# baldhat/yolov10-3D

Measured on AMD Instinct MI355X. Metric: train_images_per_sec, higher is better.
Workload: dtype bf16

## Files before the change

include/y3d.h:

```cpp
#ifndef Y3D_H
#define Y3D_H
#include <stdint.h>

#ifdef __cplusplus
extern "C" {
#endif

enum { Y3D_F32 = 0, Y3D_BF16 = 1 };
enum { Y3D_OK = 0, Y3D_ERR_INVALID = -1, Y3D_ERR_HIP = -2 };

const char* y3d_last_error(void);
int y3d_abi_version(void);
int y3d_device_info(char* name, int name_len, int* compute_units, int* lds_bytes, int* clock_khz);

int y3d_pack_weight_fwd(int dtype, const float* w_oihw, void* out, int Cout, int Cin_g, int Cin_g_pad, int kh, int kw, void* stream);
int y3d_pack_weight_dgrad(int dtype, const float* w_oihw, void* out, int Cout, int Cin_g, int groups, int kh, int kw, void* stream);
int y3d_mt_pack_weights(int dtype, const int64_t* desc, const int* chunk_tensor, const int* chunk_off, int nchunks, int chunk, void* stream);
int y3d_mt_fp8w_quantize(const int64_t* desc, const int* row_begin, int ntensors, int nrows, void* stream);
int y3d_fp8w_dequantize(const uint8_t* codes, const float* scale, float* w, int rows, int K, void* stream);
int y3d_fp8_quantize_act(const void* x, int64_t xsw, int64_t M, int C, uint8_t* q, uint8_t* s, void* stream);
int y3d_fp8_pack_weight_fwd(const uint8_t* codes, const float* scale, int rows, int Cg, uint8_t* wq, uint8_t* ws, void* stream);
int y3d_conv3x3_fp8_ok(int B, int H, int W, int Cin, int Cout, int groups);
int y3d_conv3x3_fp8_stat_rows(int B, int H, int W);
int y3d_fp8_scale_pitch(int C);
int y3d_conv3x3_fp8_fwd(const uint8_t* xq, const uint8_t* xs, int B, int H, int W, int Cin, const uint8_t* wq, const uint8_t* ws, void* y, int64_t ysw,
                        int Cout, int groups, float* stat_partials, const float* scale, const float* shift, int act, void* stream);
int y3d_fp8_quantize_grad(const void* dy, int64_t sw, const float* scale, int64_t M, int C, uint8_t* q, uint8_t* s, void* stream);
int y3d_fp8_pack_weight_dgrad(const uint8_t* codes, int Cout, int Cin, int groups, int lo, int hi, uint8_t* wq, uint8_t* ws, void* stream);
int y3d_conv3x3_fp8_dgrad_ok(int B, int H, int W, int Cin, int Cout, int groups);
int y3d_conv3x3_fp8_dgrad(const uint8_t* dyq, const uint8_t* dys, int64_t qsw, int spitch, int lo, int hi, int B, int H, int W, const uint8_t* wq, const uint8_t* ws,
                          void* dx, int64_t dxsw, int Cin, int groups, void* stream);
int y3d_conv_kpad(int dtype, int k_total);
int y3d_conv_stat_blocks(int B, int Ho, int Wo);
int y3d_conv2d_stat_rows(int dtype, int B, int H, int W, int Cin, int Cout, int groups, int kh, int kw, int stride, int pad);
enum { Y3D_OP_FWD = 0, Y3D_OP_BWD_DATA = 1, Y3D_OP_BWD_WEIGHT = 2 };
enum { Y3D_EPI_RAW = 0, Y3D_EPI_PARTIALS = 1, Y3D_EPI_AFFINE = 2, Y3D_EPI_AFFINE_RES = 3, Y3D_EPI_BIAS = 4 };
enum {
  Y3D_ROUTE_GENERIC = 0,
  Y3D_ROUTE_STREAM1X1 = 1,
  Y3D_ROUTE_SMALL = 2,
  Y3D_ROUTE_SMALL_S2 = 3,
  Y3D_ROUTE_S2_DGRAD = 4,
  Y3D_ROUTE_TILE8 = 5,
  Y3D_ROUTE_TILE16 = 6,
  Y3D_ROUTE_WIDE3_8 = 7,
  Y3D_ROUTE_WIDE3_16 = 8,
  Y3D_ROUTE_FLAT = 9,
  Y3D_ROUTE_WGRAD_SMALL = 10,
  Y3D_ROUTE_WGRAD_TILE = 11,
  Y3D_ROUTE_WGRAD_STREAM1X1 = 12
};
int y3d_conv2d_route(int dtype, int op, int epi, int B, int H, int W, int Cin, int Cout, int groups, int kh, int kw, int stride, int pad);
int y3d_conv2d_fwd(int dtype, const void* x, int64_t xsb, int64_t xsh, int64_t xsw, int B, int H, int W, int Cin,
                   const void* w_packed, const float* bias, void* y, int64_t ysw, int Ho, int Wo, int Cout, int groups,
                   int kh, int kw, int stride, int pad, float* stat_partials, void* stream);
int y3d_conv2d_fwd_affine(int dtype, const void* x, int64_t xsb, int64_t xsh, int64_t xsw, int B, int H, int W, int Cin,
                          const void* w_packed, const float* scale, const float* shift, int act, void* y, int64_t ysw, int Ho, int Wo,
                          int Cout, int groups, int kh, int kw, int stride, int pad, void* stream);
int y3d_conv2d_fwd_affine_res_ok(int dtype, int B, int H, int W, int Cin, int Cout, int groups, int kh, int kw, int stride, int pad);
int y3d_conv2d_fwd_affine_res(int dtype, const void* x, int64_t xsb, int64_t xsh, int64_t xsw, int B, int H, int W, int Cin,
                              const void* w_packed, const float* scale, const float* shift, int act, const void* res, int64_t rsw, void* y,
                              int64_t ysw, int Ho, int Wo, int Cout, int groups, int kh, int kw, int stride, int pad, void* stream);
int y3d_conv2d_bwd_data(int dtype, const void* dy, int64_t dsb, int64_t dsh, int64_t dsw, int B, int Ho, int Wo, int Cout,
                        const void* w_packed_dgrad, void* dx, int64_t xsw, int H, int W, int Cin, int groups, int kh, int kw,
                        int stride, int pad, void* stream);
int y3d_conv2d_wgrad_splits(int dtype, int B, int Ho, int Wo, int Cout, int Cin_g, int groups, int kh, int kw);
int y3d_conv2d_wgrad_plan(int dtype, int B, int H, int W, int Cin, int Cout, int groups, int kh, int kw, int stride, int pad);
int y3d_set_tile_kernels(int enable);
int y3d_set_stream1x1(int enable);
int y3d_get_stream1x1(void);
int y3d_get_tile_kernels(void);
int y3d_set_bn_wide_slabs(int enable);
int y3d_conv2d_bwd_weight(int dtype, const void* x, int64_t xsb, int64_t xsh, int64_t xsw, int B, int H, int W, int Cin,
                          int Cin_real, const void* dy, int64_t dsw, int Ho, int Wo, int Cout, int groups, int kh, int kw,
                          int stride, int pad, float* slab, int nsplit, float* grad_oihw, int accumulate, void* stream);

int y3d_dw_blocks(int64_t M);
int y3d_dw_wgrad_blocks(int64_t M);
int y3d_dw_pack_weight(const float* w_oihw, float* out_taps_c, int C, int kh, int kw, void* stream);
int y3d_dwconv2d_fwd(int dtype, const void* x, int64_t xsb, int64_t xsh, int64_t xsw, int B, int H, int W, int C,
                     const float* w_packed, void* y, int64_t ysw, int Ho, int Wo, int kh, int kw, int stride, int pad,
                     float* stat_partials, void* stream);
int y3d_dwconv2d_fwd_affine(int dtype, const void* x, int64_t xsb, int64_t xsh, int64_t xsw, int B, int H, int W, int C,
                            const float* w_packed, const float* scale, const float* shift, int act, int res_mode, const void* res, int64_t rsw,
                            void* z, int64_t zsw, int Ho, int Wo, int kh, int kw, int stride, int pad, void* stream);
int y3d_dwconv2d_bwd_data(int dtype, const void* dy, int64_t dsb, int64_t dsh, int64_t dsw, int B, int Ho, int Wo, int C,
                          const float* w_packed, void* dx, int64_t xsw, int H, int W, int kh, int kw, int stride, int pad,
                          void* stream);
int y3d_dwconv2d_bwd_weight(int dtype, const void* x, int64_t xsb, int64_t xsh, int64_t xsw, int B, int H, int W, int C,
                            const void* dy, int64_t dsw, int Ho, int Wo, int kh, int kw, int stride, int pad, float* slab,
                            float* grad_oihw, int accumulate, void* stream);

int y3d_bn_finalize(const float* partials, int nblk, int C, int64_t count, const float* gamma, const float* beta, float eps,
                    float momentum, float* running_mean, float* running_var, float* mean, float* invstd, float* scale,
                    float* shift, void* stream);
int y3d_bn_eval_scale(int C, const float* gamma, const float* beta, const float* running_mean, const float* running_var,
                      float eps, float* scale, float* shift, void* stream);
int y3d_bn_act_fwd(int dtype, const void* y, int64_t ysw, const float* scale, const float* shift, int act, int res_mode,
                   const void* res, int64_t rsw, void* z, int64_t zsw, int64_t P, int C, void* stream);
int y3d_bn_act_fwd_q(const void* y, int64_t ysw, const float* scale, const float* shift, int act, void* z, int64_t zsw, uint8_t* q, uint8_t* s,
                     int64_t P, int C, void* stream);
int y3d_bn_bwd_blocks(int64_t P, int C);
int y3d_bn_act_bwd_reduce(int dtype, const void* y, int64_t ysw, const void* dz, int64_t dsw, const void* res, int64_t rsw,
                          const float* scale, const float* shift, const float* mean, const float* invstd, int act,
                          int res_mode, float* partials, int64_t P, int C, void* stream);
int y3d_bn_bwd_finalize(const float* partials, int nblk, int C, int64_t count, float* dgamma, float* dbeta, int accumulate,
                        float* mean_g, float* mean_gx, void* stream);
int y3d_bn_act_bwd_apply(int dtype, const void* y, int64_t ysw, const void* dz, int64_t dsw, const void* res, int64_t rsw,
                         const float* scale, const float* shift, const float* mean, const float* invstd,
                         const float* mean_g, const float* mean_gx, int act, int res_mode, int train, void* dy, int64_t dysw,
                         void* dres, int64_t drsw, int64_t P, int C, void* stream);
int y3d_colsum_partials(int dtype, const void* x, int64_t xsw, float* partials, int64_t P, int C, void* stream);

int y3d_maxpool_fwd(int dtype, const void* x, int64_t xsb, int64_t xsh, int64_t xsw, void* y, int64_t ysw, uint8_t* argmax,
                    int B, int H, int W, int C, int k, void* stream);
int y3d_maxpool_bwd(int dtype, const void* dy, int64_t dsw, const uint8_t* argmax, void* dx, int64_t xsw, int B, int H, int W,
                    int C, int k, void* stream);
int y3d_upsample2x_fwd(int dtype, const void* x, int64_t xsb, int64_t xsh, int64_t xsw, void* y, int64_t ysw, int B, int H, int W,
                       int C, void* stream);
int y3d_upsample2x_bwd(int dtype, const void* dy, int64_t dsb, int64_t dsh, int64_t dsw, void* dx, int64_t xsw, int B, int H,
                       int W, int C, void* stream);
int y3d_copy2d(int dtype, const void* x, int64_t xsw, void* y, int64_t ysw, int64_t P, int C, void* stream);
int y3d_occupy_cus(int n, const int* flag, float* buf, int64_t nbuf, void* stream);
int y3d_add2d(int dtype, const void* a, int64_t asw, const void* b, int64_t bsw, void* y, int64_t ysw, int64_t P, int C, void* stream);
int y3d_nchw_to_nhwc(int dtype, const float* x_nchw, void* y_nhwc, int B, int C, int H, int W, int Cpad, void* stream);
int y3d_stem_im2col(int dtype, const float* x_nchw, void* out, int B, int H, int W, int Ho, int Wo, void* stream);
int y3d_stem_im2col_u8(int dtype, const uint8_t* x, int hwc, void* out, int B, int H, int W, int Ho, int Wo, void* stream);
int y3d_stem_conv_eval(const void* x, int in_mode, const float* wcol, const float* scale, const float* shift, int act, void* y, int64_t ysw,
                       int B, int H, int W, int Cout, void* stream);
int y3d_stem_conv_train_rows(int B, int H, int W);
int y3d_stem_conv_train(const void* x, int in_mode, const float* wcol, void* y, int64_t ysw, void* xcol, float* part, int B, int H, int W,
                        int Cout, void* stream);
int y3d_nhwc_to_nchw(int dtype, const void* x_nhwc, int64_t xsw, float* y_nchw, int B, int C, int H, int W, void* stream);
int y3d_proj_fwd(int dtype, const void* x, int64_t xsw, const float* w, const float* bias, void* y, int64_t ysw, int64_t P,
                 int Cin, int Cout, void* stream);
int y3d_proj_bwd_data(int dtype, const void* dy, int64_t dsw, const float* w, void* dx, int64_t xsw, int64_t P, int Cin, int Cout,
                      void* stream);
int y3d_proj_blocks(int64_t P);
int y3d_proj_bwd_weight(int dtype, const void* x, int64_t xsw, const void* dy, int64_t dsw, float* slab, float* bias_slab,
                        float* grad_w, float* grad_b, int accumulate, int64_t P, int Cin, int Cout, void* stream);
int y3d_slab_reduce(const float* slab, float* out, int nblk, int64_t n, int accumulate, void* stream);
int y3d_proj_group_fwd(int dtype, int nb, int cin, const void* x, int64_t xsw, const int* xoff, const float* const* w,
                       const float* const* b, const int* couts, void* y, int64_t ysw, int64_t P, void* stream);
int y3d_proj_group_bwd_data(int dtype, int nb, int cin, const void* dy, int64_t dsw, const int* xoff, const float* const* w,
                            const int* couts, void* dx, int64_t xsw, int64_t P, void* stream);
int y3d_proj_group_fwd_bn_mfma(int nb, int cin, const void* y_pre, int64_t ysw, const int* xoff, const float* const* w, const float* const* b,
                               const int* couts, const float* scale, const float* shift, int act, void* out, int64_t osw, int64_t P,
                               void* stream);
int y3d_proj_group_bwd_weight_bn_mfma_blocks(int64_t P);
int y3d_proj_group_bwd_weight_bn_mfma(int nb, int cin, const void* y_pre, int64_t ysw, const int* xoff, const void* dout, int64_t dsw,
                                      const int* couts, const float* scale, const float* shift, int act, float* slab, float* bslab,
                                      float* const* dw, float* const* db, int64_t P, void* stream);
int y3d_proj_group_bn_bwd_blocks(int64_t P);
int y3d_proj_group_bn_bwd(int mode, int nb, int cin, const void* y_pre, int64_t ysw, const int* xoff, const void* dout, int64_t dsw,
                          const float* const* w, const int* couts, const float* scale, const float* shift, const float* mean,
                          const float* invstd, const float* mean_g, const float* mean_gx, int act, float* partials, int nblk, void* dy,
                          int64_t dysw, int64_t P, int C, void* stream);
int y3d_proj_group_blocks(int64_t P);
int y3d_proj_group_fwd_bn(int dtype, int nb, int cin, const void* y_pre, int64_t xsw, const int* xoff, const float* const* w,
                          const float* const* b, const int* couts, const float* scale, const float* shift, int act, void* out,
                          int64_t ysw, int64_t P, void* stream);
int y3d_proj_group_bwd_weight_bn(int dtype, int nb, int cin, const void* y_pre, int64_t xsw, const int* xoff, const void* dy, int64_t dsw,
                                 const int* couts, const float* scale, const float* shift, int act, float* slab, float* bslab,
                                 float* const* dw, float* const* db, int64_t P, void* stream);
int y3d_proj_group_bwd_weight(int dtype, int nb, int cin, const void* x, int64_t xsw, const int* xoff, const void* dy, int64_t dsw,
                              const int* couts, float* slab, float* bslab, float* const* dw, float* const* db, int64_t P, void* stream);

int y3d_attn_fwd(int dtype, const void* qkv, int64_t qsw, void* out, int64_t osw, float* lse, int B, int N, int nh, int kd, int hd,
                 float scale, void* stream);
int y3d_attn_bwd(int dtype, const void* qkv, int64_t qsw, const void* out, int64_t osw, const void* dout, int64_t dsw,
                 const void* dv_extra, int64_t esw, const float* lse, float* delta, void* dqkv, int64_t gsw, int B, int N, int nh,
                 int kd, int hd, float scale, void* stream);

int y3d_tal3d_scratch_floats(int B, int n, int A, int topk);
int y3d_pad_targets(const float* rows, int nbox, int width, int B, int cap, float scale_x, float scale_y, float* out, int* n_used,
                    void* stream);
int y3d_tal3d_assign(int dtype, int nl, const void* const* maps, const int64_t* psw, const int* H, const int* W, const float* strides,
                     int B, int nc, const float* gt, int n, const float* calib, const float* mean_sizes, int topk, float alpha,
                     float beta, float gamma, int mode, float* scratch, uint8_t* fg_mask, int* target_gt_idx, float* target_scores, float* scal,
                     const int* n_used, void* stream);
int y3d_loss3d(int dtype, int nl, const void* const* maps, const int64_t* psw, void* const* grads, const int64_t* gsw, const int* H,
               const int* W, const float* strides, int B, int nc, const float* gt, int n, const uint8_t* fg_mask,
               const int* target_gt_idx, const float* target_scores, const float* scal, float w_loss2d, float w_cls, float w_depth,
               float w_offset3d, float w_size3d, float w_heading, float grad_scale, float* partials, float* items, void* stream);

int y3d_distill_loss(int dtype, int nl, const void* const* embs, const int64_t* psw, const int* H, const int* W, int B, int C,
                     const void* teacher, int teacher_dtype, int th, int tw, int64_t tsb, int64_t tsc, int64_t tsh, int64_t tsw,
                     const float* gt, int n, const uint8_t* fg_mask, const int* target_gt_idx, const float* scal, const uint8_t* mixed,
                     int img_w, int img_h, float T, float weight, int criterion, int no_mixup, int cap, int* counts, int* idx,
                     void* rows, float* partials, float* loss, void* stream);
int y3d_distill_scatter(int dtype, const void* rows, const int* idx, const int* nrows, const float* scale, int cap, int C, void* grad,
                        int64_t sb, int64_t sh, int64_t sw, int a0, int H, int W, void* stream);

int y3d_tal2d_assign(int dtype, int nl, const void* const* maps, const int64_t* psw, const int* H, const int* W, const float* strides,
                     int B, int nc, const float* gt, int n, int topk, float alpha, float beta, float* scratch, uint8_t* fg_mask,
                     int* target_gt_idx, float* target_scores, float* scal, const int* n_used, void* stream);
int y3d_loss2d(int dtype, int nl, const void* const* maps, const int64_t* psw, void* const* grads, const int64_t* gsw, const int* H,
               const int* W, const float* strides, int B, int nc, const float* gt, int n, const uint8_t* fg_mask,
               const int* target_gt_idx, const float* target_scores, const float* scal, float w_box, float w_cls, float w_dfl,
               float grad_scale, float* partials, float* items, void* stream);
int y3d_tal2d_scratch_floats(int B, int n, int A, int topk);
int y3d_tal2d_assign_crowded(int dtype, int nl, const void* const* maps, const int64_t* psw, const int* H, const int* W, const float* strides,
                             int B, int nc, const float* gt, int n, int topk, float alpha, float beta, float* scratch, uint8_t* fg_mask,
                             int* target_gt_idx, float* target_scores, float* scal, const int* n_used, void* stream);

int y3d_topk_cells(int dtype, const void* cls, int64_t psw, int B, int HW, int nc, int K, int* out_idx, void* stream);
int y3d_patch_gather(int dtype, const void* x, int64_t xsb, int64_t xsh, int64_t xsw, const int* idx, void* out, int B, int H, int W,
                     int C, int K, int ps, void* stream);
int y3d_head3d_scatter(int dtype, const void* cls, int64_t csw, const void* reg, int64_t rsw, const int* idx, void* map, int B, int HW,
                       int nc, int no, int K, void* stream);
int y3d_head3d_decode(int dtype, int nl, const void* const* maps, const int* H, const int* W, const float* strides, int B, int nc,
                      float* y, void* stream);
int y3d_head2d_decode(int dtype, int nl, const void* const* maps, const int* H, const int* W, const float* strides, int B, int nc,
                      float* y, void* stream);
int y3d_v10_postprocess_scratch_floats(int B, int A, int nc, int max_det);
int y3d_v10_postprocess(const float* y, int B, int C, int A, int nc, int max_det, int boxes_first, float* reg, float* scores,
                        int64_t* labels, float* scratch, void* stream);

int y3d_kitti_image_aug(const unsigned char* const* src, const unsigned char* const* src2, const int* hw, const int* flip, const double* trans_inv,
                        int B, int out_h, int out_w, int mode, void* out, void* stream);
int y3d_kde_depth_fusion(const float* predsO, int B, int K, const float* predsM, int KM, int C, float thres, float iou_thres, int nprop,
                         float* out, void* stream);
int y3d_kitti_decode(const float* preds, int B, int K, const double* calib, const double* ratio, const double* inv_trans,
                     const double* mean_size, int nc, int use_camera_dis, double threshold, double* out, unsigned char* keep, void* stream);
int y3d_kitti_encode_labels(const double* rec, const int* img_i, const double* img_f, int B, int out_w, int out_h, double min_depth,
                            double max_depth, int use_camera_dis, const double* mean_size, int n_cls, int max_objs, int64_t* cls,
                            double* bboxes, float* center_2d, float* size_2d, double* center_3d, double* size_3d, double* depth,
                            int64_t* heading_bin, double* heading_res, float* batch_idx, int* counts, double* calib, double* ratio_pad,
                            void* stream);
int y3d_json3d_encode_labels(const double* rec, const int* img_i, const double* img_f, int B, int dataset, int out_w, int out_h,
                             double min_depth, double max_depth, int use_camera_dis, const double* mean_size, int n_cls, int max_objs,
                             int64_t* cls, double* bboxes, float* center_2d, float* size_2d, double* center_3d, double* size_3d,
                             double* depth, int64_t* heading_bin, double* heading_res, float* batch_idx, int* counts, double* calib,
                             double* ratio_pad, void* stream);
int y3d_yolo2d_image_aug(const unsigned char* const* src, int n_src, const int* rec_i, const double* rec_f, const unsigned char* lut, int B,
                         int imgsz, int mode, void* out, void* stream);
int y3d_yolo2d_encode_labels(const float* rec, int n_rec, const int* lab_i, const float* lab_f, int B, int imgsz, int cap, float* cls,
                             float* bboxes, float* batch_idx, int* counts, void* stream);

int y3d_kitti_eval_max_boxes(void);
int y3d_kitti_box_overlaps(int metric, const float* gt, const float* dt, const int* gt_off, const int* dt_off, const int64_t* ov_off,
                           int n_img, float* out, void* stream);
int y3d_kitti_eval_thresholds(const float* gt, const int* gt_code, const float* dt, const int* dt_code, const int* gt_off, const int* dt_off,
                              const int64_t* ov_off, const float* ov, int n_img, int total_gt, int metric, const int* cd, int ncd,
                              const double* min_ov, int nk, float* tp_score, int* nvalid, void* stream);
int y3d_kitti_eval_counts(const float* gt, const int* gt_code, const float* dt, const int* dt_code, const int* gt_off, const int* dt_off,
                          const int64_t* ov_off, const float* ov, int n_img, int metric, const int* cd, int ncd, const double* min_ov, int nk,
                          const float* thr, const int* nthr, int compute_aos, int* cnt, double* sim, double* pr, void* stream);

int y3d_det_metrics_max_gts(void);
int y3d_det_metrics_max_dets(void);
int y3d_box_iou(const float* box1, int n1, const float* box2, int n2, float eps, float* out, void* stream);
int y3d_match_predictions(const float* iou, const int* gt_cls, int n_gt, const int* det_cls, int n_det, const float* thr, int n_thr,
                          int* tp, void* stream);
int y3d_box_match_batch(int mode, const void* preds, const unsigned char* keep, int B, int K, const double* meta, int img_h, int img_w,
                        int single_cls, const float* gt_img, const float* gt_cls, const float* gt_box, int n_gt, const float* thr,
                        int n_thr, int* tp, double* conf, int* cls, int* status, void* stream);
int y3d_ap_per_class(const int* tp, const double* conf, const int* cls, int64_t n, const int* ucls, const double* nl, int nc, int n_thr,
                     const double* x_ap, int n_ap, const double* x_curve, int n_curve, double* ap, double* p_curve, double* r_curve,
                     void* stream);

int y3d_mt_sqnorm(const int64_t* grad_ptrs, const int64_t* sizes, const int* chunk_tensor, const int* chunk_off, int nchunks, int chunk,
                  float* partials, void* stream);
int y3d_mt_copy(const int64_t* src_ptrs, const int64_t* dst_ptrs, const int64_t* sizes, const int* chunk_tensor, const int* chunk_off,
                int nchunks, int chunk, float scale, void* stream);
int y3d_mt_clip_coef(const float* partials, int nchunks, float max_norm, float* out_norm_clip, void* stream);
int y3d_mt_sgd(const int64_t* param_ptrs, const int64_t* grad_ptrs, const int64_t* buf_ptrs, const int64_t* sizes, const float* lr,
               const float* wd, const int* chunk_tensor, const int* chunk_off, int nchunks, int chunk, float momentum, int nesterov,
               int first_step, const float* norm_clip, void* stream);

int y3d_mt_adamw(const int64_t* param_ptrs, const int64_t* grad_ptrs, const int64_t* m_ptrs, const int64_t* v_ptrs, const int64_t* sizes,
                 const float* lr, const float* wd, const int* chunk_tensor, const int* chunk_off, int nchunks, int chunk, float beta1, float beta2,
                 float eps, float bias_corr1, float bias_corr2_sqrt, const float* norm_clip, void* stream);
int y3d_mt_ema(const int64_t* ema_ptrs, const int64_t* model_ptrs, const int64_t* sizes, const int* reps, const int* chunk_tensor,
               const int* chunk_off, int nchunks, int chunk, float decay, float one_minus_decay, const float* guard, void* stream);

#ifdef __cplusplus
}
#endif
#endif
```

yolov10-3d_amd/_lib.py:

```python
from __future__ import annotations

import ctypes
import os
import re

_HERE = os.path.dirname(os.path.abspath(__file__))
LIB_PATH = os.path.join(_HERE, "liby3d_hip.so")
HEADER = os.path.join(os.path.dirname(_HERE), "include", "y3d.h")

F32, BF16 = 0, 1

_CT = {"int": ctypes.c_int, "int64_t": ctypes.c_int64, "float": ctypes.c_float, "double": ctypes.c_double}


class Y3DError(RuntimeError):
    pass


def parse_header(path: str = HEADER):
    src = open(path).read()
    src = re.sub(r"/\*.*?\*/", " ", src, flags=re.S)
    protos = {}
    for m in re.finditer(r"(const\s+char\s*\*|int)\s+(y3d_\w+)\s*\(([^;{]*?)\)\s*;", src, flags=re.S):
        ret, name, args = m.group(1), m.group(2), m.group(3).strip()
        argtypes = []
        if args and args != "void":
            for a in args.split(","):
                a = a.strip()
                if "*" in a:
                    argtypes.append(ctypes.c_void_p)
                else:
                    toks = a.split()
                    t = toks[1] if toks[0] == "const" else toks[0]
                    argtypes.append(_CT[t])
        protos[name] = (ctypes.c_char_p if "char" in ret else ctypes.c_int, argtypes)
    return protos


_PLAIN_INT = {"abi_version", "conv_kpad", "conv_stat_blocks", "conv2d_stat_rows", "conv2d_route", "conv2d_wgrad_splits", "conv2d_wgrad_plan", "set_tile_kernels", "set_stream1x1", "set_bn_wide_slabs", "get_stream1x1", "get_tile_kernels", "dw_blocks", "dw_wgrad_blocks", "bn_bwd_blocks", "proj_blocks", "proj_group_blocks", "proj_group_bn_bwd_blocks", "proj_group_bwd_weight_bn_mfma_blocks", "tal3d_scratch_floats", "tal2d_scratch_floats", "v10_postprocess_scratch_floats", "conv2d_fwd_affine_res_ok", "stem_conv_train_rows", "conv3x3_fp8_ok", "conv3x3_fp8_dgrad_ok", "conv3x3_fp8_stat_rows", "fp8_scale_pitch", "kitti_eval_max_boxes", "det_metrics_max_gts", "det_metrics_max_dets"}


class _Lib:
    def __init__(self):
        if not os.path.exists(LIB_PATH):
            raise Y3DError(
                f"{LIB_PATH} not found: build it with `python yolov10-3d_amd/csrc/build.py` "
                "(or __graft_entry__.build()). There is no CPU / PyTorch fallback for the HIP path.")
        self._dll = ctypes.CDLL(LIB_PATH)
        self.protos = parse_header()
        for name, (ret, argtypes) in self.protos.items():
            fn = getattr(self._dll, name)
            fn.restype = ret
            fn.argtypes = argtypes

    def last_error(self) -> str:
        return (self._dll.y3d_last_error() or b"").decode()

    def __getattr__(self, name):
        if name.startswith("_"):
            raise AttributeError(name)
        fn = getattr(self._dll, "y3d_" + name)
        ret = self.protos["y3d_" + name][0]
        if ret is not ctypes.c_int or name in _PLAIN_INT:
            setattr(self, name, fn)
            return fn

        def call(*a):
            rc = fn(*a)
            if rc != 0:
                raise Y3DError(f"y3d_{name} failed ({rc}): {self.last_error()}")
            return rc

        setattr(self, name, call)
        return call


_lib = None


def lib() -> _Lib:
    global _lib
    if _lib is None:
        _lib = _Lib()
    return _lib
```

yolov10-3d_amd/csrc/dwconv.hip:

```cpp
#include "common.h"

namespace {

template <int CE>
__device__ __forceinline__ void pk_fma(float* acc, const float* a, const float* b) {
  typedef float f32x2_t __attribute__((ext_vector_type(2)));
#pragma unroll
  for (int j = 0; j < CE; j += 2) {
    const f32x2_t c2 = {acc[j], acc[j + 1]}, a2 = {a[j], a[j + 1]}, b2 = {b[j], b[j + 1]};
    const f32x2_t o2 = __builtin_elementwise_fma(a2, b2, c2);
    acc[j] = o2[0];
    acc[j + 1] = o2[1];
  }
}

struct DwP {
  const void* x;
  const float* w;
  void* y;
  float* part;
  long xsb, xsh, xsw, ysw;
  int B, Hg, Wg, Hq, Wq, C, kh, kw, stride, pad;
  long M;
  int px_per_block;
  const float *scale, *shift;
  const void* res;
  long rsw;
  int act, res_mode;
};

template <typename T, bool DGRAD, int K, bool AFF = false>
__global__ __launch_bounds__(256) void dwconv_kernel(DwP p) {
  constexpr int CE = TT<T>::CE;
  constexpr int CT = 64 / CE;
  constexpr int PT = 256 / CT;
  extern __shared__ __attribute__((aligned(16))) char smem[];
  float* sw = (float*)smem;
  const int taps = p.kh * p.kw;
  float* sred = sw + taps * 64;
  const int ct = threadIdx.x % CT, pt = threadIdx.x / CT;
  const int cs = blockIdx.y * 64;
  const int c = cs + ct * CE;
  for (int i = threadIdx.x; i < taps * 64; i += 256) {
    int t = i / 64, cc = i % 64;
    sw[i] = (cs + cc < p.C) ? p.w[(long)t * p.C + cs + cc] : 0.f;
  }
  __syncthreads();
  const T* __restrict__ X = (const T*)p.x;
  T* __restrict__ Y = (T*)p.y;
  float s1[CE], s2[CE];
#pragma unroll
  for (int j = 0; j < CE; ++j) { s1[j] = 0.f; s2[j] = 0.f; }
  float esc[CE], esf[CE];
  if (AFF && c < p.C) {
#pragma unroll
    for (int j = 0; j < CE; ++j) { esc[j] = p.scale[c + j]; esf[j] = p.shift[c + j]; }
  }
  if (c < p.C) {
    long pbeg = (long)blockIdx.x * p.px_per_block;
    long pend = pbeg + p.px_per_block < p.M ? pbeg + p.px_per_block : p.M;
    const int HWq = p.Hq * p.Wq;
    for (long m = pbeg + pt; m < pend; m += PT) {
      const int mi = (int)m;
      int b = mi / HWq;
      int rem = mi - b * HWq;
      int hq = rem / p.Wq, wq = rem - hq * p.Wq;
      float acc[CE];
#pragma unroll
      for (int j = 0; j < CE; ++j) acc[j] = 0.f;
      const T* xb = X + (long)b * p.xsb + c;
      if (K == 3 && DGRAD && p.stride == 2) {
        const int r0 = (hq + p.pad) & 1, q0 = (wq + p.pad) & 1;
        uint4 raw[2][2];
        int tapi[2][2];
#pragma unroll
        for (int rr = 0; rr < 2; ++rr) {
          const int r = r0 + 2 * rr, th = hq + p.pad - r, hh = th >> 1;
          const bool okh = r < 3 && th >= 0 && hh < p.Hg;
#pragma unroll
          for (int qq = 0; qq < 2; ++qq) {
            const int q = q0 + 2 * qq, tw = wq + p.pad - q, ww = tw >> 1;
            const bool ok = okh && q < 3 && tw >= 0 && ww < p.Wg;
            raw[rr][qq] = ok ? *(const uint4*)(xb + (long)hh * p.xsh + (long)ww * p.xsw) : make_uint4(0, 0, 0, 0);
            tapi[rr][qq] = ok ? r * 3 + q : 0;
          }
        }
#pragma unroll
        for (int rr = 0; rr < 2; ++rr)
#pragma unroll
          for (int qq = 0; qq < 2; ++qq) {
            float v[CE];
            Chunk<T>::unpack(raw[rr][qq], v);
            pk_fma<CE>(acc, v, sw + tapi[rr][qq] * 64 + ct * CE);
          }
      } else if (K > 0) {
#pragma unroll K == 3 ? 3 : 1
        for (int r = 0; r < K; ++r) {
          int hh;
          bool okh;
          if (DGRAD) { int t = hq + p.pad - r; hh = t / p.stride; okh = t >= 0 && hh * p.stride == t && hh < p.Hg; }
          else { hh = hq * p.stride - p.pad + r; okh = hh >= 0 && hh < p.Hg; }
          uint4 raw[K > 0 ? K : 1];
#pragma unroll
          for (int q = 0; q < K; ++q) {
            int ww;
            bool okw;
            if (DGRAD) { int t = wq + p.pad - q; ww = t / p.stride; okw = t >= 0 && ww * p.stride == t && ww < p.Wg; }
            else { ww = wq * p.stride - p.pad + q; okw = ww >= 0 && ww < p.Wg; }
            raw[q] = (okh && okw) ? *(const uint4*)(xb + (long)hh * p.xsh + (long)ww * p.xsw) : make_uint4(0, 0, 0, 0);
          }
#pragma unroll
          for (int q = 0; q < K; ++q) {
            float v[CE];
            Chunk<T>::unpack(raw[q], v);
            pk_fma<CE>(acc, v, sw + (r * K + q) * 64 + ct * CE);
          }
        }
      } else
      for (int r = 0; r < p.kh; ++r) {
        int hh;
        bool okh;
        if (DGRAD) { int t = hq + p.pad - r; hh = t / p.stride; okh = t >= 0 && hh * p.stride == t && hh < p.Hg; }
        else { hh = hq * p.stride - p.pad + r; okh = hh >= 0 && hh < p.Hg; }
        if (!okh) continue;
        for (int q = 0; q < p.kw; ++q) {
          int ww;
          bool okw;
          if (DGRAD) { int t = wq + p.pad - q; ww = t / p.stride; okw = t >= 0 && ww * p.stride == t && ww < p.Wg; }
          else { ww = wq * p.stride - p.pad + q; okw = ww >= 0 && ww < p.Wg; }
          if (!okw) continue;
          float v[CE];
          Chunk<T>::unpack(*(const uint4*)(xb + (long)hh * p.xsh + (long)ww * p.xsw), v);
          pk_fma<CE>(acc, v, sw + (r * p.kw + q) * 64 + ct * CE);
        }
      }
#pragma unroll
      for (int j = 0; j < CE; ++j) {
        acc[j] = TT<T>::rnd(acc[j]);
        s1[j] += acc[j];
        s2[j] += acc[j] * acc[j];
      }
      if (AFF) {
        float r[CE];
        if (p.res_mode) Chunk<T>::unpack(*(const uint4*)((const T*)p.res + m * p.rsw + c), r);
#pragma unroll
        for (int j = 0; j < CE; ++j) {
          float u = acc[j] * esc[j] + esf[j];
          if (p.res_mode == 2) u += r[j];
          if (p.act) u = silu_f(u);
          if (p.res_mode == 1) u += r[j];
          acc[j] = u;
        }
      }
      *(uint4*)(Y + m * p.ysw + c) = Chunk<T>::pack(acc);
    }
  }
  if (p.part) {
#pragma unroll
    for (int j = 0; j < CE; ++j) { sred[(pt * 64 + ct * CE + j) * 2] = s1[j]; sred[(pt * 64 + ct * CE + j) * 2 + 1] = s2[j]; }
    __syncthreads();
    if (threadIdx.x < 64 && cs + threadIdx.x < p.C) {
      float a = 0.f, b2 = 0.f;
      for (int r = 0; r < PT; ++r) { a += sred[(r * 64 + threadIdx.x) * 2]; b2 += sred[(r * 64 + threadIdx.x) * 2 + 1]; }
      p.part[((long)blockIdx.x * p.C + cs + threadIdx.x) * 2] = a;
      p.part[((long)blockIdx.x * p.C + cs + threadIdx.x) * 2 + 1] = b2;
    }
  }
}

struct DwWP {
  const void* x;
  const void* dy;
  float* slab;
  long xsb, xsh, xsw, dsw;
  int B, H, W, Ho, Wo, C, kh, kw, stride, pad;
  long M;
  int px_per_block, nblk, nslab;
};

template <typename T, int K>
__global__ __launch_bounds__(256) void dwconv_wgrad_kernel(DwWP p) {
  constexpr int CE = TT<T>::CE;
  constexpr int CT = 64 / CE;
  constexpr int PT = 256 / CT;
  constexpr int RP = 1;
  constexpr int KW = K > 0 ? K : 8;
  __shared__ float sh[4][RP * KW * 64];
  const int ct = threadIdx.x % CT, pt = threadIdx.x / CT;
  const int kh = K > 0 ? K : p.kh, kw = K > 0 ? K : p.kw;
  const int L = blockIdx.x, jx = L >> 3;
  const int row = jx % kh, tile = (jx / kh) * 8 + (L & 7);
  if (tile >= p.nblk * p.nslab) return;
  const int bx = tile % p.nblk;
  const int cs = (tile / p.nblk) * 64;
  const int c = cs + ct * CE;
  const int taps = kh * kw;
  const T* __restrict__ X = (const T*)p.x;
  const T* __restrict__ D = (const T*)p.dy;
  const long pbeg = (long)bx * p.px_per_block;
  const long pend = pbeg + p.px_per_block < p.M ? pbeg + p.px_per_block : p.M;
  const int HWo = p.Ho * p.Wo;
  {
    const int r0 = row * RP;
    float acc[RP][KW][CE];
#pragma unroll
    for (int r = 0; r < RP; ++r)
#pragma unroll
      for (int q = 0; q < KW; ++q)
#pragma unroll
        for (int j = 0; j < CE; ++j) acc[r][q][j] = 0.f;
    if (c < p.C) {
      long m = pbeg + pt;
      int b = (int)(m / HWo);
      int rem = (int)(m - (long)b * HWo);
      int ho = rem / p.Wo, wo = rem - ho * p.Wo;
      auto one = [&](const uint4& dv, int bb, int hh0, int ww0) {
        float d[CE];
        Chunk<T>::unpack(dv, d);
        const T* xb = X + (long)bb * p.xsb + c;
        uint4 raw[RP][KW];
#pragma unroll
        for (int r = 0; r < RP; ++r) {
          const int hh = hh0 + r0 + r;
          const bool okh = r0 + r < kh && hh >= 0 && hh < p.H;
#pragma unroll
          for (int q = 0; q < KW; ++q) {
            const int ww = ww0 + q;
            const bool ok = okh && q < kw && ww >= 0 && ww < p.W;
            raw[r][q] = ok ? *(const uint4*)(xb + (long)hh * p.xsh + (long)ww * p.xsw) : make_uint4(0, 0, 0, 0);
          }
        }
#pragma unroll
        for (int r = 0; r < RP; ++r)
#pragma unroll
          for (int q = 0; q < KW; ++q) {
            float v[CE];
            Chunk<T>::unpack(raw[r][q], v);
            pk_fma<CE>(acc[r][q], d, v);
          }
      };
      auto advance = [&]() {
        wo += PT;
        while (wo >= p.Wo) { wo -= p.Wo; ++ho; }
        while (ho >= p.Ho) { ho -= p.Ho; ++b; }
      };
      for (; m + PT < pend; m += 2 * PT) {
        const uint4 d0 = *(const uint4*)(D + m * p.dsw + c), d1 = *(const uint4*)(D + (m + PT) * p.dsw + c);
        const int b0 = b, h0 = ho * p.stride - p.pad, w0 = wo * p.stride - p.pad;
        advance();
        const int b1 = b, h1 = ho * p.stride - p.pad, w1 = wo * p.stride - p.pad;
        advance();
        one(d0, b0, h0, w0);
        one(d1, b1, h1, w1);
      }
      if (m < pend) one(*(const uint4*)(D + m * p.dsw + c), b, ho * p.stride - p.pad, wo * p.stride - p.pad);
    }
    const int lane = threadIdx.x & 63, wave = threadIdx.x >> 6;
#pragma unroll
    for (int r = 0; r < RP; ++r)
#pragma unroll
      for (int q = 0; q < KW; ++q)
#pragma unroll
        for (int j = 0; j < CE; ++j) {
          float v = acc[r][q][j];
          if (CT == 8) v = lane_xor8_sum(v);
          v = lane_xor32_sum(lane_xor16_sum(v));
          if (lane < CT) sh[wave][(r * KW + q) * 64 + ct * CE + j] = v;
        }
    __syncthreads();
    for (int i = threadIdx.x; i < RP * KW * 64; i += 256) {
      const int t = i >> 6, cc = i & 63;
      const int r = t / KW, q = t - r * KW;
      if (r0 + r < kh && q < kw && cs + cc < p.C)
        p.slab[((long)bx * taps + (r0 + r) * kw + q) * p.C + cs + cc] = sh[0][i] + sh[1][i] + sh[2][i] + sh[3][i];
    }
  }
}

__global__ __launch_bounds__(256) void dw_wgrad_reduce_kernel(const float* __restrict__ slab, float* __restrict__ grad, int nblk, int taps, int C,
                                                              int accumulate) {
  __shared__ float sh[8][32];
  const int e = threadIdx.x & 31, sl = threadIdx.x >> 5;
  const int idx = blockIdx.x * 32 + e;
  const int n = taps * C;
  float s = 0.f;
  if (idx < n)
    for (int b = sl; b < nblk; b += 8) s += slab[(long)b * n + idx];
  sh[sl][e] = s;
  __syncthreads();
  if (sl != 0 || idx >= n) return;
#pragma unroll
  for (int j = 1; j < 8; ++j) s += sh[j][e];
  const int c = idx % C, t = idx / C;
  const long o = (long)c * taps + t;
  grad[o] = accumulate ? grad[o] + s : s;
}

__global__ void dw_pack_kernel(const float* __restrict__ w, float* __restrict__ out, int C, int taps) {
  int idx = blockIdx.x * blockDim.x + threadIdx.x;
  if (idx >= taps * C) return;
  int c = idx % C, t = idx / C;
  out[idx] = w[(long)c * taps + t];
}

}

extern "C" {

int y3d_dw_blocks(int64_t M) {
  long n = (M + 63) / 64;
  return (int)(n < 1 ? 1 : (n > 2048 ? 2048 : n));
}

int y3d_dw_wgrad_blocks(int64_t M) {
  long n = (M + 127) / 128;
  return (int)(n < 1 ? 1 : (n > 1024 ? 1024 : n));
}

int y3d_dw_pack_weight(const float* w_oihw, float* out, int C, int kh, int kw, void* stream) {
  hipLaunchKernelGGL(dw_pack_kernel, dim3(cdiv((long)C * kh * kw, 256)), dim3(256), 0, (hipStream_t)stream, w_oihw, out, C, kh * kw);
  Y3D_LAUNCH_CHECK();
  return Y3D_OK;
}

#define DW_LAUNCH_K(T, D, K) hipLaunchKernelGGL((dwconv_kernel<T, D, K>), grid, dim3(256), sm, st, p)
#define DW_LAUNCH_A(T, K) hipLaunchKernelGGL((dwconv_kernel<T, false, K, true>), grid, dim3(256), sm, st, p)
#define DW_LAUNCH(T)                                                                                             \
  do {                                                                                                           \
    const int kk = (p.kh == p.kw && (p.kh == 3 || p.kh == 7)) ? p.kh : 0;                                        \
    if (!dgrad && p.scale) { if (kk == 3) DW_LAUNCH_A(T, 3); else if (kk == 7) DW_LAUNCH_A(T, 7); else DW_LAUNCH_A(T, 0); }           \
    else if (dgrad) { if (kk == 3) DW_LAUNCH_K(T, true, 3); else if (kk == 7) DW_LAUNCH_K(T, true, 7); else DW_LAUNCH_K(T, true, 0); }     \
    else { if (kk == 3) DW_LAUNCH_K(T, false, 3); else if (kk == 7) DW_LAUNCH_K(T, false, 7); else DW_LAUNCH_K(T, false, 0); }        \
  } while (0)

static int dw_launch(int dtype, bool dgrad, const DwP& p, hipStream_t st) {
  Y3D_CHECK(p.M < (1L << 31), "dwconv: more than 2^31 pixels");
  int ce = dtype == Y3D_BF16 ? 8 : 4;
  int pt = 256 / (64 / ce);
  size_t sm = (size_t)(p.kh * p.kw * 64 + pt * 64 * 2) * sizeof(float);
  dim3 grid(y3d_dw_blocks(p.M), cdiv(p.C, 64));
  if (dtype == Y3D_BF16) {
    DW_LAUNCH(bf16_t);
  } else {
    DW_LAUNCH(float);
  }
  Y3D_LAUNCH_CHECK();
  return Y3D_OK;
}

int y3d_dwconv2d_fwd(int dtype, const void* x, int64_t xsb, int64_t xsh, int64_t xsw, int B, int H, int W, int C,
                     const float* w_packed, void* y, int64_t ysw, int Ho, int Wo, int kh, int kw, int stride, int pad,
                     float* stat_partials, void* stream) {
  int ce = dtype == Y3D_BF16 ? 8 : 4;
  Y3D_CHECK(dtype == Y3D_BF16 || dtype == Y3D_F32, "dwconv2d_fwd: bad dtype");
  Y3D_CHECK(C % ce == 0, "dwconv2d_fwd: C=%d not a multiple of %d", C, ce);
  Y3D_CHECK(Ho == (H + 2 * pad - kh) / stride + 1 && Wo == (W + 2 * pad - kw) / stride + 1, "dwconv2d_fwd: output dims");
  Y3D_CHECK((((uintptr_t)x | (uintptr_t)y) & 15) == 0 && xsb % ce == 0 && xsh % ce == 0 && xsw % ce == 0 && ysw % ce == 0, "dwconv2d_fwd: alignment");
  DwP p;
  p.x = x; p.w = w_packed; p.y = y; p.part = stat_partials;
  p.scale = nullptr; p.shift = nullptr; p.res = nullptr; p.rsw = 0; p.act = 0; p.res_mode = 0;
  p.xsb = xsb; p.xsh = xsh; p.xsw = xsw; p.ysw = ysw;
  p.B = B; p.Hg = H; p.Wg = W; p.Hq = Ho; p.Wq = Wo; p.C = C; p.kh = kh; p.kw = kw; p.stride = stride; p.pad = pad;
  p.M = (long)B * Ho * Wo;
  int nblk = y3d_dw_blocks(p.M);
  p.px_per_block = (int)((p.M + nblk - 1) / nblk);
  return dw_launch(dtype, false, p, (hipStream_t)stream);
}

int y3d_dwconv2d_fwd_affine(int dtype, const void* x, int64_t xsb, int64_t xsh, int64_t xsw, int B, int H, int W, int C,
                            const float* w_packed, const float* scale, const float* shift, int act, int res_mode, const void* res, int64_t rsw,
                            void* z, int64_t zsw, int Ho, int Wo, int kh, int kw, int stride, int pad, void* stream) {
  int ce = dtype == Y3D_BF16 ? 8 : 4;
  Y3D_CHECK(dtype == Y3D_BF16 || dtype == Y3D_F32, "dwconv2d_fwd_affine: bad dtype");
  Y3D_CHECK(C % ce == 0, "dwconv2d_fwd_affine: C=%d not a multiple of %d", C, ce);
  Y3D_CHECK(Ho == (H + 2 * pad - kh) / stride + 1 && Wo == (W + 2 * pad - kw) / stride + 1, "dwconv2d_fwd_affine: output dims");
  Y3D_CHECK((((uintptr_t)x | (uintptr_t)z) & 15) == 0 && xsb % ce == 0 && xsh % ce == 0 && xsw % ce == 0 && zsw % ce == 0, "dwconv2d_fwd_affine: alignment");
  Y3D_CHECK(scale && shift && res_mode >= 0 && res_mode <= 2, "dwconv2d_fwd_affine: scale / shift missing or bad residual mode");
  Y3D_CHECK(res_mode == 0 || (res && (((uintptr_t)res) & 15) == 0 && rsw % ce == 0), "dwconv2d_fwd_affine: residual missing or misaligned");
  DwP p;
  p.x = x; p.w = w_packed; p.y = z; p.part = nullptr;
  p.scale = scale; p.shift = shift; p.res = res; p.rsw = rsw; p.act = act; p.res_mode = res_mode;
  p.xsb = xsb; p.xsh = xsh; p.xsw = xsw; p.ysw = zsw;
  p.B = B; p.Hg = H; p.Wg = W; p.Hq = Ho; p.Wq = Wo; p.C = C; p.kh = kh; p.kw = kw; p.stride = stride; p.pad = pad;
  p.M = (long)B * Ho * Wo;
  int nblk = y3d_dw_blocks(p.M);
  p.px_per_block = (int)((p.M + nblk - 1) / nblk);
  return dw_launch(dtype, false, p, (hipStream_t)stream);
}

int y3d_dwconv2d_bwd_data(int dtype, const void* dy, int64_t dsb, int64_t dsh, int64_t dsw, int B, int Ho, int Wo, int C,
                          const float* w_packed, void* dx, int64_t xsw, int H, int W, int kh, int kw, int stride, int pad,
                          void* stream) {
  int ce = dtype == Y3D_BF16 ? 8 : 4;
  Y3D_CHECK(dtype == Y3D_BF16 || dtype == Y3D_F32, "dwconv2d_bwd_data: bad dtype");
  Y3D_CHECK(C % ce == 0, "dwconv2d_bwd_data: C=%d not a multiple of %d", C, ce);
  Y3D_CHECK((((uintptr_t)dy | (uintptr_t)dx) & 15) == 0 && dsb % ce == 0 && dsh % ce == 0 && dsw % ce == 0 && xsw % ce == 0, "dwconv2d_bwd_data: alignment");
  DwP p;
  p.x = dy; p.w = w_packed; p.y = dx; p.part = nullptr;
  p.scale = nullptr; p.shift = nullptr; p.res = nullptr; p.rsw = 0; p.act = 0; p.res_mode = 0;
  p.xsb = dsb; p.xsh = dsh; p.xsw = dsw; p.ysw = xsw;
  p.B = B; p.Hg = Ho; p.Wg = Wo; p.Hq = H; p.Wq = W; p.C = C; p.kh = kh; p.kw = kw; p.stride = stride; p.pad = pad;
  p.M = (long)B * H * W;
  int nblk = y3d_dw_blocks(p.M);
  p.px_per_block = (int)((p.M + nblk - 1) / nblk);
  return dw_launch(dtype, true, p, (hipStream_t)stream);
}

int y3d_dwconv2d_bwd_weight(int dtype, const void* x, int64_t xsb, int64_t xsh, int64_t xsw, int B, int H, int W, int C,
                            const void* dy, int64_t dsw, int Ho, int Wo, int kh, int kw, int stride, int pad, float* slab,
                            float* grad_oihw, int accumulate, void* stream) {
  int ce = dtype == Y3D_BF16 ? 8 : 4;
  Y3D_CHECK(dtype == Y3D_BF16 || dtype == Y3D_F32, "dwconv2d_bwd_weight: bad dtype");
  Y3D_CHECK(C % ce == 0, "dwconv2d_bwd_weight: C=%d not a multiple of %d", C, ce);
  Y3D_CHECK((((uintptr_t)x | (uintptr_t)dy) & 15) == 0 && xsb % ce == 0 && xsh % ce == 0 && xsw % ce == 0 && dsw % ce == 0, "dwconv2d_bwd_weight: alignment");
  DwWP p;
  p.x = x; p.dy = dy; p.slab = slab;
  p.xsb = xsb; p.xsh = xsh; p.xsw = xsw; p.dsw = dsw;
  p.B = B; p.H = H; p.W = W; p.Ho = Ho; p.Wo = Wo; p.C = C; p.kh = kh; p.kw = kw; p.stride = stride; p.pad = pad;
  p.M = (long)B * Ho * Wo;
  int nblk = y3d_dw_wgrad_blocks(p.M);
  p.px_per_block = (int)((p.M + nblk - 1) / nblk);
  p.nblk = nblk; p.nslab = cdiv(C, 64);
  dim3 grid(cdiv(nblk * p.nslab, 8) * 8 * kh);
  hipStream_t st = (hipStream_t)stream;
  Y3D_CHECK(kw <= 8 || (kh == kw && (kh == 3 || kh == 7)), "dwconv2d_bwd_weight: kernels wider than 8 taps are not supported");
#define Y3D_DWW(T)                                                                                                          \
  do {                                                                                                                      \
    if (kh == 3 && kw == 3) hipLaunchKernelGGL((dwconv_wgrad_kernel<T, 3>), grid, dim3(256), 0, st, p);                      \
    else if (kh == 7 && kw == 7) hipLaunchKernelGGL((dwconv_wgrad_kernel<T, 7>), grid, dim3(256), 0, st, p);                 \
    else hipLaunchKernelGGL((dwconv_wgrad_kernel<T, 0>), grid, dim3(256), 0, st, p);                                         \
  } while (0)
  if (dtype == Y3D_BF16) Y3D_DWW(bf16_t); else Y3D_DWW(float);
#undef Y3D_DWW
  Y3D_LAUNCH_CHECK();
  hipLaunchKernelGGL(dw_wgrad_reduce_kernel, dim3(cdiv((long)C * kh * kw, 32)), dim3(256), 0, st, slab, grad_oihw, nblk, kh * kw, C, accumulate);
  Y3D_LAUNCH_CHECK();
  return Y3D_OK;
}

}
```

yolov10-3d_amd/ops.py:

```python
from __future__ import annotations

import os
from collections import namedtuple

import torch

from ._lib import BF16, F32, Y3DError, lib

_COMPUTE_DTYPE = torch.bfloat16


def set_compute_dtype(dt: torch.dtype):
    global _COMPUTE_DTYPE
    if dt not in (torch.bfloat16, torch.float32):
        raise ValueError("compute dtype must be torch.bfloat16 or torch.float32")
    _COMPUTE_DTYPE = dt


def compute_dtype() -> torch.dtype:
    return _COMPUTE_DTYPE


def code(dt: torch.dtype) -> int:
    if dt == torch.bfloat16:
        return BF16
    if dt == torch.float32:
        return F32
    raise Y3DError(f"unsupported tensor dtype {dt}")


def ce(dt: torch.dtype) -> int:
    return 8 if dt == torch.bfloat16 else 4


def stream() -> int:
    return torch.cuda.current_stream().cuda_stream


def _require_gpu(x: torch.Tensor):
    if not x.is_cuda:
        raise Y3DError("the y3d HIP path needs tensors on a HIP device (there is no CPU fallback)")


def nhwc_empty(B, C, H, W, dtype, device):
    return torch.empty((B, H, W, C), dtype=dtype, device=device).permute(0, 3, 1, 2)


PLACEMENT = True
EVAL_LEVEL_STREAMS = True
_LEVEL_STREAMS: list = []


def level_streams(n: int):
    while len(_LEVEL_STREAMS) < n:
        _LEVEL_STREAMS.append(torch.cuda.Stream())
    return _LEVEL_STREAMS[:n]
_PLACE = None


class place:

    def __init__(self, buf, off):
        self.t = (buf, off) if buf is not None else None

    def __enter__(self):
        global _PLACE
        self.prev, _PLACE = _PLACE, self.t

    def __exit__(self, *a):
        global _PLACE
        _PLACE = self.prev


_PLACE_FINAL = None


class place_final:
    def __init__(self, buf, off):
        self.t = (buf, off) if buf is not None else None

    def __enter__(self):
        global _PLACE_FINAL
        self.prev, _PLACE_FINAL = _PLACE_FINAL, self.t

    def __exit__(self, *a):
        global _PLACE_FINAL
        _PLACE_FINAL = self.prev


def final_place():
    global _PLACE_FINAL
    t, _PLACE_FINAL = _PLACE_FINAL, None
    return place(*(t or (None, 0)))


def concat_buffer(x, C, H=None, W=None):
    dtype = _COMPUTE_DTYPE
    if not PLACEMENT or not x.is_cuda or C % ce(dtype) != 0:
        return None
    buf = nhwc_empty(x.shape[0], C, x.shape[2] if H is None else H, x.shape[3] if W is None else W, dtype, x.device)
    _CONCAT_BASE[buf.data_ptr()] = (C, buf)
    return buf


_CONCAT_BASE = {}


_GRAD_SLOT = {}


def grad_slot(x):
    ent = _GRAD_SLOT.get((x.data_ptr(), x.shape[1]))
    if ent is None:
        return None
    holder, off = ent
    if holder["shape"] != (x.shape[0], x.shape[2], x.shape[3]) or holder["dtype"] != x.dtype:
        return None
    return holder, off, x.shape[1]


def grad_slot_tensor(slot):
    holder, off, w = slot
    if holder["buf"] is None:
        B, H, W = holder["shape"]
        holder["buf"] = nhwc_empty(B, holder["C"], H, W, holder["dtype"], holder["device"])
    return holder["buf"][:, off:off + w]


def reset_placement():
    global _PLACE, _PLACE_FINAL
    _PLACE = None
    _PLACE_FINAL = None
    _CONCAT_BASE.clear()
    _GRAD_SLOT.clear()
    _FP8_ACT.clear()


def out_tensor(B, C, H, W, dtype, device):
    global _PLACE
    if _PLACE is not None:
        buf, off = _PLACE
        if (buf.dtype == dtype and buf.shape[0] == B and buf.shape[2] == H and buf.shape[3] == W and off + C <= buf.shape[1]
                and off % ce(dtype) == 0 and C % ce(dtype) == 0 and buf.device == device):
            _PLACE = None
            return buf[:, off:off + C]
    return nhwc_empty(B, C, H, W, dtype, device)


def is_nhwc(x: torch.Tensor) -> bool:
    return x.dim() == 4 and (x.stride(1) == 1 or x.shape[1] == 1)


def px_dense(x: torch.Tensor) -> bool:
    B, C, H, W = x.shape
    sw = x.stride(3)
    return is_nhwc(x) and sw >= C and (H == 1 or x.stride(2) == W * sw) and (B == 1 or x.stride(0) == H * W * sw)


def to_nhwc(x: torch.Tensor, dtype=None, dense=False) -> torch.Tensor:
    dtype = dtype or _COMPUTE_DTYPE
    c = ce(dtype)
    ok = (x.dtype == dtype and is_nhwc(x) and x.data_ptr() % 16 == 0 and x.stride(0) % c == 0 and x.stride(2) % c == 0
          and x.stride(3) % c == 0 and (not dense or px_dense(x)))
    if ok:
        return x
    B, C, H, W = x.shape
    out = nhwc_empty(B, C, H, W, dtype, x.device)
    out.copy_(x)
    return out


def s3(x):
    return x.stride(0), x.stride(2), x.stride(3)


def _f32(n, device):
    return torch.empty(n, dtype=torch.float32, device=device)


class KernelTimer:

    def __init__(self, want):
        self.want = want
        self.pending = []

    def bracket(self, key, fn):
        if not self.want(key):
            return fn()
        a, b = torch.cuda.Event(enable_timing=True), torch.cuda.Event(enable_timing=True)
        a.record()
        r = fn()
        b.record()
        self.pending.append((key, a, b))
        return r

    def results(self):
        torch.cuda.synchronize()
        out = {}
        for key, a, b in self.pending:
            out.setdefault(key, []).append(a.elapsed_time(b))
        return out


TIMER = None

PARAM_EPOCH = 0


def bump_param_epoch():
    global PARAM_EPOCH
    PARAM_EPOCH += 1


WEIGHT_EPOCH = 0


def bump_weight_epoch():
    global WEIGHT_EPOCH
    WEIGHT_EPOCH += 1
    bump_param_epoch()


class _WeightRegistry:

    KEEP = 4

    def __init__(self):
        self.entries, self.epoch, self.tables = {}, None, None
        self.captured_tables = []

    def _hold_tables(self):
        if torch.cuda.is_current_stream_capturing() and not any(t is self.tables for t in self.captured_tables):
            self.captured_tables.append(self.tables)

    def _revisit(self, e, now, ver, refresh_all):
        e["seen"] = WEIGHT_EPOCH
        capturing = torch.cuda.is_current_stream_capturing()
        if capturing:
            e["pinned"] = True
        if self.epoch != now:
            self.epoch = now
            stale = [] if capturing else [k for k, v in self.entries.items() if WEIGHT_EPOCH - v["seen"] > self.KEEP and not v.get("pinned")]
            for k in stale:
                del self.entries[k]
            for v in refresh_all():
                v["ver"] = None
        changed = e["ver"] is not None and e["ver"] != ver
        e["ver"] = ver
        return changed


class _PackRegistry(_WeightRegistry):

    CHUNK = 16384

    def __init__(self, mode):
        super().__init__()
        self.mode = mode

    def _pack_one(self, e):
        L, st = lib(), stream()
        a, b, c, taps, kpad, dt = e["geo"]
        k = int(round(taps ** 0.5))
        if self.mode == 0:
            L.pack_weight_fwd(dt, e["src"], e["dst"].data_ptr(), a, b, c, k, k, st)
        else:
            L.pack_weight_dgrad(dt, e["src"], e["dst"].data_ptr(), a * b, c, a, k, k, st)

    def _pack_all(self, dt):
        ents = [e for e in self.entries.values() if e["geo"][5] == dt]
        if not ents:
            return ents
        dev = ents[0]["dst"].device
        key = tuple(id(e) for e in ents)
        if self.tables is None or self.tables[0] != (key, dt):
            desc, ct, co = [], [], []
            for t, e in enumerate(ents):
                a, b, c, taps, kpad, _ = e["geo"]
                n = a * kpad if self.mode == 0 else a * c * kpad
                desc += [e["src"], e["dst"].data_ptr(), a, b, c, taps, kpad, self.mode]
                for j in range((n + self.CHUNK - 1) // self.CHUNK):
                    ct.append(t)
                    co.append(j)
            self.tables = ((key, dt), torch.tensor(desc, dtype=torch.int64, device=dev), torch.tensor(ct, dtype=torch.int32, device=dev),
                           torch.tensor(co, dtype=torch.int32, device=dev), len(ct))
        _, desc, ct, co, n = self.tables
        self._hold_tables()
        lib().mt_pack_weights(dt, desc.data_ptr(), ct.data_ptr(), co.data_ptr(), n, self.CHUNK, stream())
        return ents

    def lookup(self, w32, src_ptr, geo, dtype, ver=None):
        key = (src_ptr, geo)
        ver = w32._version if ver is None else ver
        e = self.entries.get(key)
        if e is None:
            a, b, c, taps, kpad, dt = geo
            n = a * kpad if self.mode == 0 else a * c * kpad
            e = {"src": src_ptr, "geo": geo, "dst": torch.empty(n, dtype=dtype, device=w32.device), "ver": ver, "seen": WEIGHT_EPOCH,
                 "keep": w32}
            self.entries[key] = e
            self._pack_one(e)
        elif self._revisit(e, (WEIGHT_EPOCH, geo[5]), ver, lambda: self._pack_all(geo[5])):
            self._pack_one(e)
        return e["dst"]


class _QuantRegistry(_WeightRegistry):

    def _run(self, ents):
        dev = ents[0]["weff"].device
        key = tuple(id(e) for e in ents)
        if self.tables is None or self.tables[0] != key:
            desc, rb, r = [], [], 0
            for e in ents:
                rows, K = e["shape"]
                desc += [e["src"], e["weff"].data_ptr(), e["codes"].data_ptr(), e["scale"].data_ptr(), rows, K]
                rb.append(r)
                r += rows
            self.tables = (key, torch.tensor(desc, dtype=torch.int64, device=dev), torch.tensor(rb, dtype=torch.int32, device=dev), len(ents), r)
        _, desc, rb, nt, nrows = self.tables
        self._hold_tables()
        lib().mt_fp8w_quantize(desc.data_ptr(), rb.data_ptr(), nt, nrows, stream())
        return ents

    def _run_one(self, e):
        tb, self.tables = self.tables, None
        self._run([e])
        self.tables = tb

    def lookup(self, w32, ver=None):
        ver = w32._version if ver is None else ver
        rows, K = w32.shape[0], w32[0].numel()
        key = (w32.data_ptr(), rows, K)
        e = self.entries.get(key)
        if e is None:
            dev = w32.device
            e = {"src": w32.data_ptr(), "shape": (rows, K), "keep": w32, "weff": torch.empty(w32.shape, dtype=torch.float32, device=dev),
                 "codes": torch.empty((rows, K), dtype=torch.uint8, device=dev), "scale": torch.empty(rows, dtype=torch.float32, device=dev),
                 "ver": ver, "count": 0, "seen": WEIGHT_EPOCH}
            self.entries[key] = e
            self._run_one(e)
        elif self._revisit(e, WEIGHT_EPOCH, ver, lambda: self._run(list(self.entries.values()))):
            e["count"] += 1
            self._run_one(e)
        self.last = e
        return e["weff"], (WEIGHT_EPOCH, e["count"])


PACK_FWD, PACK_DGRAD, QUANT = _PackRegistry(0), _PackRegistry(1), _QuantRegistry()
WEIGHT_QUANT = None


def set_weight_quant(mode):
    global WEIGHT_QUANT
    if mode not in (None, "fp8"):
        raise ValueError("weight quantisation mode must be None or 'fp8'")
    WEIGHT_QUANT = mode
    if mode is None:
        set_fp8_dgrad(False)
    bump_param_epoch()


def weight_quant():
    return WEIGHT_QUANT


FP8_CONV = False
FP8_DGRAD = False
_FP8_WANT = False
_FP8_ACT = {}


def set_fp8_conv(on: bool):
    global FP8_CONV
    if on and WEIGHT_QUANT != "fp8":
        raise ValueError('set_fp8_conv(True) needs set_weight_quant("fp8"): the kernel multiplies the fp8w quantiser\'s codes')
    FP8_CONV = bool(on)
    if not on:
        set_fp8_dgrad(False)
    bump_param_epoch()


def fp8_conv():
    return FP8_CONV


def set_fp8_dgrad(on: bool):
    global FP8_DGRAD
    if on and not FP8_CONV:
        raise ValueError("set_fp8_dgrad(True) needs set_fp8_conv(True): the data gradient follows the layers whose forward runs in fp8")
    FP8_DGRAD = bool(on)


def fp8_dgrad():
    return FP8_DGRAD


class want_fp8_copy:

    def __enter__(self):
        global _FP8_WANT
        self.prev, _FP8_WANT = _FP8_WANT, FP8_CONV
        return self

    def __exit__(self, *a):
        global _FP8_WANT
        _FP8_WANT = self.prev


def fp8_input(xin):
    B, C, H, W = xin.shape
    ent = _FP8_ACT.pop(xin.data_ptr(), None)
    if ent is not None and ent[2] == (B, C, H, W):
        return ent[0], ent[1]
    if not px_dense(xin):
        xin = to_nhwc(xin, torch.bfloat16, dense=True).contiguous(memory_format=torch.channels_last)
    q = torch.empty(B, H, W, C, dtype=torch.uint8, device=xin.device)
    s = torch.empty(B, H, W, lib().fp8_scale_pitch(C), dtype=torch.uint8, device=xin.device)
    lib().fp8_quantize_act(xin.data_ptr(), xin.stride(3), B * H * W, C, q.data_ptr(), s.data_ptr(), stream())
    return q, s


def fp8_weight(ent, Cg):
    tok = (WEIGHT_EPOCH, ent["count"])
    hit = ent.get("wq")
    if hit is None or hit[0] != tok:
        rows = ent["shape"][0]
        dev = ent["codes"].device
        wq = hit[1] if hit is not None else torch.empty(rows, 9, Cg, dtype=torch.uint8, device=dev)
        ws = hit[2] if hit is not None else torch.empty(rows, dtype=torch.uint8, device=dev)
        lib().fp8_pack_weight_fwd(ent["codes"].data_ptr(), ent["scale"].data_ptr(), rows, Cg, wq.data_ptr(), ws.data_ptr(), stream())
        hit = ent["wq"] = (tok, wq, ws)
    return hit[1], hit[2]


def fp8_weight_dgrad(ent, Cin, g, lo, hi):
    tok = (WEIGHT_EPOCH, ent["count"])
    cache = ent.setdefault("wqd", {})
    hit = cache.get((g, lo, hi))
    if hit is None or hit[0] != tok:
        Cout = ent["shape"][0]
        dev = ent["codes"].device
        wq = hit[1] if hit is not None else torch.empty(g, Cin // g, 9, (hi - lo) // g, dtype=torch.uint8, device=dev)
        ws = hit[2] if hit is not None else torch.empty(Cin, dtype=torch.uint8, device=dev)
        lib().fp8_pack_weight_dgrad(ent["codes"].data_ptr(), Cout, Cin, g, lo, hi, wq.data_ptr(), ws.data_ptr(), stream())
        hit = cache[(g, lo, hi)] = (tok, wq, ws)
    return hit[1], hit[2]


PROJ_BN_MFMA = True
STEM_FUSED = True
PACK_CACHE = True
DW_EVAL_FUSED = True


def conv_bn_act_eval(x, w, gamma, beta, rm, rv, k, s, p, g, act, eps, cache=None, ver=None):
    z, _, _ = _cba_forward(x, w, gamma, beta, rm, rv, k, s, p, g, act, None, 0, False, eps, 0.0, cache, ver=ver)
    return z


_IDENT = {}


def _identity_bn(C, device):
    ident = _IDENT.get((C, device))
    if ident is None:
        ident = _IDENT[(C, device)] = (torch.ones(C, dtype=torch.float32, device=device), torch.zeros(C, dtype=torch.float32, device=device))
    return ident


def conv_bias_act_eval(x, w, bias, k, s, p, g, act, res, res_mode, cache):
    _require_gpu(x)
    ones, zeros = _identity_bn(w.shape[0], w.device)
    with torch.no_grad():
        z, _, _ = _cba_forward(x, _w32(w), ones, bias.detach().float(), zeros, ones, k, s, p, g, act, res, res_mode, False, 0.0, 0.0, cache)
    return z


def _cache_put(cache, key, value):
    for old in [q for q in cache if q[1] != PARAM_EPOCH]:
        del cache[old]
    cache[key] = value


def _eval_consts(cache, kind, w32, g32, b32, rm, rv, ver, dtype, k, g, Cin_g, Cg_pad, Cout, eps):
    L, st, dev = lib(), stream(), w32.device
    vkey = ver[1] if ver is not None else (w32._version, g32._version, b32._version, rm._version, rv._version)
    key = (kind, PARAM_EPOCH, w32.data_ptr(), g32.data_ptr(), rm.data_ptr(), vkey, dtype, k, g, Cg_pad, Cout, float(eps))
    hit = cache.get(key) if cache is not None else None
    if hit is None:
        if kind == "dw":
            wp = _f32(k * k * Cout, dev)
            L.dw_pack_weight(w32.data_ptr(), wp.data_ptr(), Cout, k, k, st)
        else:
            wp = torch.empty(Cout * k * k * Cg_pad, dtype=dtype, device=dev)
            L.pack_weight_fwd(code(dtype), w32.data_ptr(), wp.data_ptr(), Cout, Cin_g, Cg_pad, k, k, st)
        ss = _f32(2 * Cout, dev).view(2, Cout)
        L.bn_eval_scale(Cout, g32.data_ptr(), b32.data_ptr(), rm.data_ptr(), rv.data_ptr(), eps, ss[0].data_ptr(), ss[1].data_ptr(), st)
        hit = (wp, ss, w32)
        if cache is not None:
            _cache_put(cache, key, hit)
    return hit[0], hit[1]


def _timed(key, launch):
    if TIMER is not None:
        TIMER.bracket(key, launch)
    else:
        launch()


ConvPlan = namedtuple("ConvPlan", "B Cin Cin_k H W Cout Ho Wo k s p g dw res_mode training dtype act wver fp8_entry stem", defaults=(False,))


def _cba_forward(x, w32, g32, b32, rm, rv, k, s, p, g, act, res, res_mode, training, eps, momentum, cache=None, bn_apply=True, ver=None):
    _require_gpu(x)
    dtype = _COMPUTE_DTYPE
    B, Cin, H, W = x.shape
    dw = g > 1 and g == Cin and g == w32.shape[0]
    qent = None
    if WEIGHT_QUANT and not dw:
        w32, qtok = QUANT.lookup(w32, ver[0] if ver is not None else None)
        qent = QUANT.last
        ver = ((qtok,), (qtok,) + (ver[1] if ver is not None else (g32._version, b32._version, rm._version, rv._version)))
    Cout, Cg_w, kh, kw = w32.shape
    assert kh == k and kw == k and Cin // g == Cg_w, "Conv: weight shape does not match input"
    if Cin == 3 and k == 3 and s == 2 and p == 1 and g == 1 and not x.requires_grad:
        return _stem_forward(x, w32, g32, b32, rm, rv, act, res, res_mode, training, eps, momentum, cache, ver)
    c = ce(dtype)
    if Cin % c != 0:
        if g != 1:
            raise Y3DError(f"grouped conv with {Cin} channels is not 16-byte chunkable")
        Cin_k = (Cin + c - 1) // c * c
        xin = nhwc_empty(B, Cin_k, H, W, dtype, x.device)
        lib().nchw_to_nhwc(code(dtype), x.float().contiguous().data_ptr(), xin.data_ptr(), B, Cin, H, W, Cin_k, stream())
    else:
        xin = to_nhwc(x, dtype)
    if dw:
        return _dw_forward(xin, w32, g32, b32, rm, rv, k, s, p, act, res, res_mode, training, eps, momentum, cache, bn_apply, ver)
    return _dense_forward(xin, w32, g32, b32, rm, rv, Cin, k, s, p, g, act, res, res_mode, training, eps, momentum, cache, bn_apply, ver, qent, True)


def _stem_image(x):
    if x.dtype == torch.uint8:
        hwc = int(not x.is_contiguous() and x.permute(0, 2, 3, 1).is_contiguous())
        return (x if (hwc or x.is_contiguous()) else x.contiguous()), hwc
    return x.float().contiguous(), 0


def _stem_forward(x, w32, g32, b32, rm, rv, act, res, res_mode, training, eps, momentum, cache, ver):
    L, st, dtype, dev = lib(), stream(), _COMPUTE_DTYPE, x.device
    dt = code(dtype)
    B, _, H, W = x.shape
    Cout = w32.shape[0]
    Ho, Wo = (H - 1) // 2 + 1, (W - 1) // 2 + 1
    wkey = ("stemcol", PARAM_EPOCH, w32.data_ptr(), ver[0] if ver is not None else w32._version)
    wcol = cache.get(wkey) if (cache is not None and not training) else None
    if wcol is None:
        wcol = torch.zeros(Cout, 32, dtype=torch.float32, device=dev)
        wcol[:, :27] = w32.detach().permute(0, 2, 3, 1).reshape(Cout, 27)
        if cache is not None and not training:
            _cache_put(cache, wkey, wcol)
    w1x1 = wcol.view(Cout, 32, 1, 1)
    fused = dtype == torch.bfloat16 and Cout % 16 == 0 and 16 <= Cout <= 80 and STEM_FUSED and x.dtype in (torch.uint8, torch.float32)
    if fused and not training and not res_mode:
        _, ss = _eval_consts(cache, "dense", w1x1, g32, b32, rm, rv, ver, dtype, 1, 1, 32, 32, Cout, eps)
        xs, hwc = _stem_image(x)
        mode = 1 + hwc if xs.dtype == torch.uint8 else 0
        ye = out_tensor(B, Cout, Ho, Wo, dtype, dev)
        _timed(("conv_eval", dt, B, H, W, 3, Cout, 3, 2, 1, 1),
               lambda: L.stem_conv_eval(xs.data_ptr(), mode, wcol.data_ptr(), ss[0].data_ptr(), ss[1].data_ptr(), int(act), ye.data_ptr(), ye.stride(3),
                                        B, H, W, Cout, st))
        return ye, None, None
    xcol = nhwc_empty(B, 32, Ho, Wo, dtype, dev)
    xs, hwc = _stem_image(x)
    if fused and training:
        mode = 1 + hwc if xs.dtype == torch.uint8 else 0
        rows = L.stem_conv_train_rows(B, H, W)
        ypre = nhwc_empty(B, Cout, Ho, Wo, dtype, dev)
        part = _f32(rows * Cout * 2, dev)
        _timed(("conv_fwd", dt, B, H, W, 3, Cout, 3, 2, 1),
               lambda: L.stem_conv_train(xs.data_ptr(), mode, wcol.data_ptr(), ypre.data_ptr(), ypre.stride(3), xcol.data_ptr(), part.data_ptr(), B, H, W, Cout, st))
        z, plan, saved = _bn_act_tail(xcol, w1x1, ypre, part, rows, None, g32, b32, rm, rv, 32, 1, 1, 0, 1, act, res, res_mode, training, eps, momentum,
                                      True, None, None)
    else:
        if xs.dtype == torch.uint8:
            L.stem_im2col_u8(dt, xs.data_ptr(), hwc, xcol.data_ptr(), B, H, W, Ho, Wo, st)
        else:
            L.stem_im2col(dt, xs.data_ptr(), xcol.data_ptr(), B, H, W, Ho, Wo, st)
        z, plan, saved = _dense_forward(xcol, w1x1, g32, b32, rm, rv, 32, 1, 1, 0, 1, act, res, res_mode, training, eps, momentum, cache, True, None,
                                        None, False)
    return z, (plan._replace(stem=True) if plan is not None else None), saved


def _dw_forward(xin, w32, g32, b32, rm, rv, k, s, p, act, res, res_mode, training, eps, momentum, cache, bn_apply, ver):
    L, st, dtype, dev = lib(), stream(), xin.dtype, xin.device
    dt = code(dtype)
    B, C, H, W = xin.shape
    Ho, Wo = (H + 2 * p - k) // s + 1, (W + 2 * p - k) // s + 1
    sb, sh, sw = s3(xin)
    fused = not training and bn_apply and DW_EVAL_FUSED
    y = None if fused else nhwc_empty(B, C, Ho, Wo, dtype, dev)
    nblk = L.dw_blocks(B * Ho * Wo)
    part = ss_eval = None
    if training:
        part = _f32(nblk * C * 2, dev)
        wp = _f32(k * k * C, dev)
        L.dw_pack_weight(w32.data_ptr(), wp.data_ptr(), C, k, k, st)
    else:
        wp, ss_eval = _eval_consts(cache, "dw", w32, g32, b32, rm, rv, ver, dtype, k, C, 1, 1, C, eps)
        if fused:
            ze = out_tensor(B, C, Ho, Wo, dtype, dev)
            rr = to_nhwc(res, dtype, dense=True) if res_mode else None
            if rr is not None:
                assert rr.shape == ze.shape, "residual shape mismatch"
            L.dwconv2d_fwd_affine(dt, xin.data_ptr(), sb, sh, sw, B, H, W, C, wp.data_ptr(), ss_eval[0].data_ptr(), ss_eval[1].data_ptr(), int(act),
                                  res_mode, rr.data_ptr() if rr is not None else None, rr.stride(3) if rr is not None else 0,
                                  ze.data_ptr(), ze.stride(3), Ho, Wo, k, k, s, p, st)
            return ze, None, None
    L.dwconv2d_fwd(dt, xin.data_ptr(), sb, sh, sw, B, H, W, C, wp.data_ptr(), y.data_ptr(), C, Ho, Wo, k, k, s, p,
                   part.data_ptr() if training else None, st)
    return _bn_act_tail(xin, w32, y, part, nblk, ss_eval, g32, b32, rm, rv, C, k, s, p, C, act, res, res_mode, training, eps, momentum, bn_apply,
                        ver[0] if ver is not None else None, None)


def _dense_forward(xin, w32, g32, b32, rm, rv, Cin, k, s, p, g, act, res, res_mode, training, eps, momentum, cache, bn_apply, ver, qent, pack_cache):
    L, st, dtype, dev = lib(), stream(), xin.dtype, xin.device
    dt = code(dtype)
    B, Cin_k, H, W = xin.shape
    Cout = w32.shape[0]
    Ho, Wo = (H + 2 * p - k) // s + 1, (W + 2 * p - k) // s + 1
    sb, sh, sw = s3(xin)
    wver = ver[0] if ver is not None else None
    y = nhwc_empty(B, Cout, Ho, Wo, dtype, dev) if (training or res_mode) else None
    f8 = (FP8_CONV and qent is not None and dtype == torch.bfloat16 and k == 3 and s == 1 and p == 1 and Cin_k == Cin
          and bool(L.conv3x3_fp8_ok(B, H, W, Cin, Cout, g)))
    nblk = L.conv3x3_fp8_stat_rows(B, H, W) if f8 else L.conv2d_stat_rows(dt, B, H, W, Cin_k, Cout, g, k, k, s, p)
    part = _f32(nblk * Cout * 2, dev) if training else None
    Cg_pad = Cin_k // g
    wp = ss_eval = None
    if not training:
        wp, ss_eval = _eval_consts(cache, "dense", w32, g32, b32, rm, rv, ver, dtype, k, g, Cin // g, Cg_pad, Cout, eps)
    if f8:
        xq, xs = fp8_input(xin)
        wq, ws = fp8_weight(qent, Cin // g)
        if not training and not res_mode:
            ye = out_tensor(B, Cout, Ho, Wo, dtype, dev)
            _timed(("conv_eval_fp8", dt, B, H, W, Cin_k, Cout, k, s, g, p),
                   lambda: L.conv3x3_fp8_fwd(xq.data_ptr(), xs.data_ptr(), B, H, W, Cin, wq.data_ptr(), ws.data_ptr(), ye.data_ptr(), ye.stride(3), Cout, g, None,
                                             ss_eval[0].data_ptr(), ss_eval[1].data_ptr(), int(act), st))
            return ye, None, None
        _timed(("conv_fwd_fp8", dt, B, H, W, Cin_k, Cout, k, s, g),
               lambda: L.conv3x3_fp8_fwd(xq.data_ptr(), xs.data_ptr(), B, H, W, Cin, wq.data_ptr(), ws.data_ptr(), y.data_ptr(), y.stride(3), Cout, g,
                                         part.data_ptr() if training else None, None, None, 0, st))
    elif not training and not res_mode:
        ye = out_tensor(B, Cout, Ho, Wo, dtype, dev)
        _timed(("conv_eval", dt, B, H, W, Cin_k, Cout, k, s, g, p),
               lambda: L.conv2d_fwd_affine(dt, xin.data_ptr(), sb, sh, sw, B, H, W, Cin_k, wp.data_ptr(), ss_eval[0].data_ptr(), ss_eval[1].data_ptr(),
                                           int(act), ye.data_ptr(), ye.stride(3), Ho, Wo, Cout, g, k, k, s, p, st))
        return ye, None, None
    elif (not training and res_mode == 1 and dtype == torch.bfloat16
            and L.conv2d_fwd_affine_res_ok(dt, B, H, W, Cin_k, Cout, g, k, k, s, p)):
        rr = to_nhwc(res, dtype, dense=True)
        ye = out_tensor(B, Cout, Ho, Wo, dtype, dev)
        L.conv2d_fwd_affine_res(dt, xin.data_ptr(), sb, sh, sw, B, H, W, Cin_k, wp.data_ptr(), ss_eval[0].data_ptr(), ss_eval[1].data_ptr(), int(act),
                                rr.data_ptr(), rr.stride(3), ye.data_ptr(), ye.stride(3), Ho, Wo, Cout, g, k, k, s, p, st)
        return ye, None, None
    else:
        if training and pack_cache and PACK_CACHE:
            wp = PACK_FWD.lookup(w32, w32.data_ptr(), (Cout, Cin // g, Cg_pad, k * k, k * k * Cg_pad, dt), dtype, wver)
        elif training:
            wp = torch.empty(Cout * k * k * Cg_pad, dtype=dtype, device=dev)
            L.pack_weight_fwd(dt, w32.data_ptr(), wp.data_ptr(), Cout, Cin // g, Cg_pad, k, k, st)
        _timed(("conv_fwd", dt, B, H, W, Cin_k, Cout, k, s, g),
               lambda: L.conv2d_fwd(dt, xin.data_ptr(), sb, sh, sw, B, H, W, Cin_k, wp.data_ptr(), None, y.data_ptr(), Cout, Ho, Wo, Cout, g,
                                    k, k, s, p, part.data_ptr() if training else None, st))
    return _bn_act_tail(xin, w32, y, part, nblk, ss_eval, g32, b32, rm, rv, Cin, k, s, p, g, act, res, res_mode, training, eps, momentum, bn_apply,
                        wver, qent if f8 else None)


def _bn_act_tail(xin, w32, y, part, nblk, ss_eval, g32, b32, rm, rv, Cin, k, s, p, g, act, res, res_mode, training, eps, momentum, bn_apply, wver,
                 fp8_entry):
    L, st, dtype, dev = lib(), stream(), y.dtype, y.device
    dt = code(dtype)
    B, Cin_k, H, W = xin.shape
    _, Cout, Ho, Wo = y.shape
    M = B * Ho * Wo
    plan = ConvPlan(B, Cin, Cin_k, H, W, Cout, Ho, Wo, k, s, p, g, g > 1 and g == Cin and g == Cout, res_mode, training, dtype, int(act), wver,
                    fp8_entry)
    if training:
        stats = _f32(6 * Cout, dev).view(6, Cout)
        bump_param_epoch()
        L.bn_finalize(part.data_ptr(), nblk, Cout, M, g32.data_ptr(), b32.data_ptr(), eps, momentum, rm.data_ptr(), rv.data_ptr(),
                      stats[0].data_ptr(), stats[1].data_ptr(), stats[2].data_ptr(), stats[3].data_ptr(), st)
    elif not bn_apply:
        stats = torch.zeros(6, Cout, dtype=torch.float32, device=dev)
        stats[2:4].copy_(ss_eval)
    else:
        stats = None
    if not bn_apply:
        return y, plan, (xin, w32, y, stats, None)
    z = out_tensor(B, Cout, Ho, Wo, dtype, dev)
    rr = None
    if res_mode:
        rr = to_nhwc(res, dtype, dense=True)
        assert rr.shape == z.shape, "residual shape mismatch"
    sc_t, sh_t = (stats[2], stats[3]) if training else (ss_eval[0], ss_eval[1])
    if _FP8_WANT and dtype == torch.bfloat16 and not res_mode and Cout % 64 == 0 and not plan.dw:
        zq = torch.empty(B, Ho, Wo, Cout, dtype=torch.uint8, device=dev)
        zs = torch.empty(B, Ho, Wo, L.fp8_scale_pitch(Cout), dtype=torch.uint8, device=dev)
        L.bn_act_fwd_q(y.data_ptr(), Cout, sc_t.data_ptr(), sh_t.data_ptr(), int(act), z.data_ptr(), z.stride(3), zq.data_ptr(), zs.data_ptr(), M, Cout, st)
        _FP8_ACT[z.data_ptr()] = (zq, zs, (B, Cout, Ho, Wo), z)
    else:
        L.bn_act_fwd(dt, y.data_ptr(), Cout, sc_t.data_ptr(), sh_t.data_ptr(), int(act), res_mode,
                     rr.data_ptr() if rr is not None else None, rr.stride(3) if rr is not None else 0, z.data_ptr(), z.stride(3), M, Cout, st)
    return z, plan, (xin, w32, y, stats, rr if res_mode == 2 else None)


def _cba_backward(plan, saved, dz, need_dx, need_dres, dx_range=None, pre=None, dx_out=None):
    L = lib()
    _, _, y, stats, rr = saved
    B, Cout, Ho, Wo, res_mode, dtype, act = plan.B, plan.Cout, plan.Ho, plan.Wo, plan.res_mode, plan.dtype, plan.act
    if not plan.training:
        raise Y3DError("backward through an eval-mode (running-statistics) Conv is not supported")
    if pre is not None:
        return _conv_backward(plan, saved, pre[0], pre[1], None, need_dx, dx_range, dx_out)
    dt, st, dev = code(dtype), stream(), dz.device
    M = B * Ho * Wo
    dz = to_nhwc(dz, dtype, dense=True)
    nb = L.bn_bwd_blocks(M, Cout)
    part = _f32(nb * Cout * 2, dev)
    rptr = rr.data_ptr() if rr is not None else None
    rsw = rr.stride(3) if rr is not None else 0
    L.bn_act_bwd_reduce(dt, y.data_ptr(), Cout, dz.data_ptr(), dz.stride(3), rptr, rsw, stats[2].data_ptr(), stats[3].data_ptr(),
                        stats[0].data_ptr(), stats[1].data_ptr(), act, res_mode, part.data_ptr(), M, Cout, st)
    dgb = _f32(2 * Cout, dev).view(2, Cout)
    L.bn_bwd_finalize(part.data_ptr(), nb, Cout, M, dgb[0].data_ptr(), dgb[1].data_ptr(), 0, stats[4].data_ptr(), stats[5].data_ptr(), st)
    dy = nhwc_empty(B, Cout, Ho, Wo, dtype, dev)
    dres = None
    if res_mode == 2 and need_dres:
        dres = nhwc_empty(B, Cout, Ho, Wo, dtype, dev)
    L.bn_act_bwd_apply(dt, y.data_ptr(), Cout, dz.data_ptr(), dz.stride(3), rptr, rsw, stats[2].data_ptr(), stats[3].data_ptr(),
                       stats[0].data_ptr(), stats[1].data_ptr(), stats[4].data_ptr(), stats[5].data_ptr(), act, res_mode, 1,
                       dy.data_ptr(), Cout, dres.data_ptr() if dres is not None else None, Cout, M, Cout, st)
    if res_mode == 1:
        dres = dz
    return _conv_backward(plan, saved, dy, dgb, dres, need_dx, dx_range, dx_out)


def _fp8_dgrad_plan(plan, need_dx, dx_range):
    ent = plan.fp8_entry
    if not (FP8_DGRAD and FP8_CONV and need_dx) or ent is None or plan.wver != ((WEIGHT_EPOCH, ent["count"]),):
        return None
    Cin, Cout, g = plan.Cin, plan.Cout, plan.g
    lo, hi = dx_range if dx_range is not None else (0, Cout)
    if plan.Cin_k != Cin or plan.dtype != torch.bfloat16 or (plan.k, plan.s, plan.p) != (3, 1, 1) or (g != 1 and (lo, hi) != (0, Cout)):
        return None
    if (lo, hi) != (0, Cout) and (lo % 128 or (hi - lo) % 128):
        return None
    if not lib().conv3x3_fp8_dgrad_ok(plan.B, plan.H, plan.W, Cin, hi - lo, g):
        return None
    return ent, lo, hi


def _conv_backward(plan, saved, dy, dgb, dres, need_dx, dx_range, dx_out=None):
    L = lib()
    xin, w32 = saved[:2]
    B, Cin, Cin_k, H, W, Cout, Ho, Wo = plan.B, plan.Cin, plan.Cin_k, plan.H, plan.W, plan.Cout, plan.Ho, plan.Wo
    k, s, p, g, dtype = plan.k, plan.s, plan.p, plan.g, plan.dtype
    dt, st = code(dtype), stream()
    dev = dy.device
    esz = 2 if dtype == torch.bfloat16 else 4
    M = B * Ho * Wo
    sb, sh, sw = s3(xin)
    dx = None
    dW = torch.empty_like(w32)
    if plan.dw:
        wp = _f32(k * k * Cout, dev)
        L.dw_pack_weight(w32.data_ptr(), wp.data_ptr(), Cout, k, k, st)
        if need_dx:
            dx = nhwc_empty(B, Cin, H, W, dtype, dev)
            dsb, dsh, dsw = s3(dy)
            L.dwconv2d_bwd_data(dt, dy.data_ptr(), dsb, dsh, dsw, B, Ho, Wo, Cout, wp.data_ptr(), dx.data_ptr(), Cin, H, W, k, k, s, p, st)
        slab = _f32(L.dw_wgrad_blocks(M) * k * k * Cout, dev)
        L.dwconv2d_bwd_weight(dt, xin.data_ptr(), sb, sh, sw, B, H, W, Cin, dy.data_ptr(), Cout, Ho, Wo, k, k, s, p, slab.data_ptr(),
                              dW.data_ptr(), 0, st)
    else:
        f8 = _fp8_dgrad_plan(plan, need_dx, dx_range)
        if f8 is not None and not (px_dense(dy) and dy.data_ptr() % 16 == 0 and dy.stride(3) % 8 == 0):
            f8 = None
        if f8 is not None:
            qent, lo, hi = f8
            wqd, wsd = fp8_weight_dgrad(qent, Cin, g, lo, hi)
            co = hi - lo
            dq = torch.empty(B, Ho, Wo, co, dtype=torch.uint8, device=dev)
            ds = torch.empty(B, Ho, Wo, L.fp8_scale_pitch(co), dtype=torch.uint8, device=dev)
            L.fp8_quantize_grad(dy.data_ptr() + lo * esz, dy.stride(3), qent["scale"].data_ptr() + lo * 4, M, co, dq.data_ptr(), ds.data_ptr(), st)
            dx = dx_out if dx_out is not None else nhwc_empty(B, Cin, H, W, dtype, dev)
            if not (px_dense(dx) and dx.data_ptr() % 16 == 0 and dx.stride(3) % 8 == 0):
                raise Y3DError("fp8 data gradient: dx must be a pixel-dense NHWC tensor with 16-byte aligned rows")
            _timed(("conv_dgrad_fp8", dt, B, H, W, Cin, hi - lo, k, s, g),
                   lambda: L.conv3x3_fp8_dgrad(dq.data_ptr(), ds.data_ptr(), co, ds.shape[3], 0, co, B, H, W, wqd.data_ptr(), wsd.data_ptr(),
                                               dx.data_ptr(), dx.stride(3), Cin, g, st))
        elif need_dx and Cin_k == Cin:
            lo, hi = dx_range if dx_range is not None else (0, Cout)
            assert g == 1 or (lo, hi) == (0, Cout)
            co = hi - lo
            kp = L.conv_kpad(dt, k * k * (co // g))
            src = w32.data_ptr() + lo * (Cin // g) * k * k * 4
            if plan.stem or not PACK_CACHE:
                wpd = torch.empty(Cin * kp, dtype=dtype, device=dev)
                L.pack_weight_dgrad(dt, src, wpd.data_ptr(), co, Cin // g, g, k, k, st)
            else:
                wpd = PACK_DGRAD.lookup(w32, src, (g, co // g, Cin // g, k * k, kp, dt), dtype, plan.wver)
            dx = dx_out if dx_out is not None else nhwc_empty(B, Cin, H, W, dtype, dev)
            dsb, dsh, dsw = s3(dy)
            _timed(("conv_dgrad", dt, B, H, W, Cin, co, k, s, g),
                   lambda: L.conv2d_bwd_data(dt, dy.data_ptr() + lo * esz, dsb, dsh, dsw, B, Ho, Wo, co, wpd.data_ptr(), dx.data_ptr(), dx.stride(3), H, W,
                                             Cin, g, k, k, s, p, st))
        ns = L.conv2d_wgrad_plan(dt, B, H, W, Cin_k, Cout, g, k, k, s, p)
        slab = _f32(ns * Cout * k * k * (Cin_k // g), dev)
        _timed(("conv_wgrad", dt, B, H, W, Cin_k, Cout, k, s, g),
               lambda: L.conv2d_bwd_weight(dt, xin.data_ptr(), sb, sh, sw, B, H, W, Cin_k, Cin, dy.data_ptr(), Cout, Ho, Wo, Cout, g, k, k,
                                           s, p, slab.data_ptr(), ns, dW.data_ptr(), 0, st))
    if plan.stem:
        dW = dW.reshape(Cout, 32)[:, :27].reshape(Cout, 3, 3, 3).permute(0, 3, 1, 2).contiguous()
        dx = None
    return dx, dW, dgb[0], dgb[1], dres


def _w32(weight):
    w = weight.detach()
    if w.dtype != torch.float32 or not w.is_contiguous():
        w = w.float().contiguous()
    return w


class ConvBNActFn(torch.autograd.Function):

    @staticmethod
    def forward(ctx, x, weight, gamma, beta, res, res_mode, m):
        z, cfg, saved = _cba_forward(x, _w32(weight), gamma.detach().float(), beta.detach().float(), m.bn.running_mean, m.bn.running_var,
                                     m.k, m.s, m.p, m.g, m.has_act, res, res_mode, m.training, m.eps, m.momentum,
                                     m.__dict__.setdefault("_eval_cache", {}))
        if m.training:
            m._nbt_pending += 1
        ctx.cfg = cfg
        if saved is not None:
            ctx.save_for_backward(*saved)
        return z

    @staticmethod
    def backward(ctx, dz):
        if ctx.cfg is None:
            raise Y3DError("backward through an eval-mode (running-statistics) Conv is not supported")
        dx, dW, dg, db, dres = _cba_backward(ctx.cfg, ctx.saved_tensors, dz, ctx.needs_input_grad[0], ctx.needs_input_grad[4])
        return dx, dW, dg, db, dres, None, None


class StackedConvs:

    def __init__(self, convs, groups=1):
        self.convs = list(convs)
        self.groups = groups
        self.couts = [c.conv.out_channels for c in self.convs]
        self.flat = {}

    def _ensure(self, name, tensors, setter):
        flat = self.flat.get(name)
        ok = flat is not None and flat.device == tensors[0].device
        if ok:
            base, off = flat.data_ptr(), 0
            for t in tensors:
                if t.data_ptr() != base + off * 4:
                    ok = False
                    break
                off += t.numel()
        if not ok:
            flat = torch.cat([t.detach().reshape(-1).float() for t in tensors])
            off = 0
            for i, t in enumerate(tensors):
                n = t.numel()
                setter(i, flat[off:off + n].view(t.shape))
                off += n
            self.flat[name] = flat
        return flat

    def tensors(self):
        cs = self.convs
        w = self._ensure("w", [c.conv.weight for c in cs], lambda i, v: setattr(cs[i].conv.weight, "data", v))
        gm = self._ensure("g", [c.bn.weight for c in cs], lambda i, v: setattr(cs[i].bn.weight, "data", v))
        bt = self._ensure("b", [c.bn.bias for c in cs], lambda i, v: setattr(cs[i].bn.bias, "data", v))
        rm = self._ensure("rm", [c.bn.running_mean for c in cs], lambda i, v: cs[i].bn._buffers.__setitem__("running_mean", v))
        rv = self._ensure("rv", [c.bn.running_var for c in cs], lambda i, v: cs[i].bn._buffers.__setitem__("running_var", v))
        c0 = cs[0].conv
        wv = tuple(c.conv.weight._version for c in cs)
        self.ver = (wv, wv + tuple(t._version for c in cs for t in (c.bn.weight, c.bn.bias, c.bn.running_mean, c.bn.running_var)))
        return w.view(sum(self.couts), c0.in_channels // c0.groups, *c0.kernel_size), gm, bt, rm, rv

    def params(self):
        return [c.conv.weight for c in self.convs] + [c.bn.weight for c in self.convs] + [c.bn.bias for c in self.convs]


class FusedConvBNActFn(torch.autograd.Function):

    @staticmethod
    def forward(ctx, x, stack, groups, dx_range, *params):
        w, gm, bt, rm, rv = stack.tensors()
        m = stack.convs[0]
        z, cfg, saved = _cba_forward(x, w, gm, bt, rm, rv, m.k, m.s, m.p, groups, m.has_act, None, 0, m.training, m.eps, m.momentum, ver=stack.ver)
        if m.training:
            for c in stack.convs:
                c._nbt_pending += 1
        ctx.cfg, ctx.couts, ctx.dx_range = cfg, stack.couts, dx_range
        ctx.gslot = grad_slot(x) if (m.training and torch.is_tensor(x) and x.is_cuda) else None
        if saved is not None:
            ctx.save_for_backward(*saved)
        return z

    @staticmethod
    def backward(ctx, dz):
        dx_out = grad_slot_tensor(ctx.gslot) if (ctx.gslot is not None and ctx.needs_input_grad[0]) else None
        dx, dW, dg, db, _ = _cba_backward(ctx.cfg, ctx.saved_tensors, dz, ctx.needs_input_grad[0], False, ctx.dx_range, dx_out=dx_out)
        dWs, dgs, dbs, off = [], [], [], 0
        for co in ctx.couts:
            dWs.append(dW[off:off + co])
            dgs.append(dg[off:off + co])
            dbs.append(db[off:off + co])
            off += co
        return (dx, None, None, None, *dWs, *dgs, *dbs)


class SplitChannelsFn(torch.autograd.Function):

    @staticmethod
    def forward(ctx, x, offs, widths):
        ctx.offs, ctx.widths, ctx.C = tuple(offs), tuple(widths), x.shape[1]
        covered = sorted(zip(offs, widths))
        ctx.dense = covered[0][0] == 0 and all(a + w == b for (a, w), (b, _) in zip(covered, covered[1:])) and covered[-1][0] + covered[-1][1] == x.shape[1]
        ctx.order = [j for _, j in sorted((o, j) for j, o in enumerate(offs))]
        outs = tuple(x[:, o:o + w] for o, w in zip(offs, widths))
        ctx.holder = None
        if ctx.dense and x.is_cuda and len(set(offs)) == len(offs) and all(o % ce(x.dtype) == 0 and w % ce(x.dtype) == 0 for o, w in zip(offs, widths)):
            ctx.holder = {"buf": None, "C": x.shape[1], "shape": (x.shape[0], x.shape[2], x.shape[3]), "dtype": x.dtype, "device": x.device}
            ctx.keys = []
            for v, o in zip(outs, offs):
                k = (v.data_ptr(), v.shape[1])
                _GRAD_SLOT[k] = (ctx.holder, o)
                ctx.keys.append(k)
        return outs

    @staticmethod
    def backward(ctx, *grads):
        ref = next(g for g in grads if g is not None)
        B, _, H, W = ref.shape
        if ctx.holder is not None:
            for k in ctx.keys:
                _GRAD_SLOT.pop(k, None)
            buf = ctx.holder["buf"]
            esz = ref.element_size()
            if buf is not None and all(g is not None and g.dtype == buf.dtype and g.data_ptr() == buf.data_ptr() + o * esz and g.shape[1] == w
                                       and g.stride() == buf[:, o:o + w].stride() for g, o, w in zip(grads, ctx.offs, ctx.widths)):
                return buf, None, None
        if ctx.dense and all(g is not None for g in grads):
            parts = [to_nhwc(grads[j], ref.dtype, dense=True).permute(0, 2, 3, 1) for j in ctx.order]
            return torch.cat(parts, 3).permute(0, 3, 1, 2), None, None
        dx = nhwc_empty(B, ctx.C, H, W, ref.dtype, ref.device)
        dx.zero_()
        for g, o, w in zip(grads, ctx.offs, ctx.widths):
            if g is not None:
                dx[:, o:o + w].add_(g)
        return dx, None, None


class InjectRowsFn(torch.autograd.Function):

    @staticmethod
    def forward(ctx, z, slot):
        ctx.slot = slot
        return z.view_as(z)

    @staticmethod
    def backward(ctx, g):
        entries = ctx.slot.pop("entries", ())
        live = [e for e in entries if e["scale"] is not None]
        if g is None or not live:
            return g, None
        dt = live[0]["rows"].dtype
        g = to_nhwc(g, dt)
        sb, sh, sw = s3(g)
        B, _, H, W = g.shape
        for e in live:
            lib().distill_scatter(code(dt), e["rows"].data_ptr(), e["idx"].data_ptr(), e["nrows"].data_ptr(), e["scale"].data_ptr(), e["cap"],
                                  e["C"], g.data_ptr() + e["off"] * g.element_size(), sb, sh, sw, e["a0"], H, W, stream())
        return g, None


class C2fSplitFn(torch.autograd.Function):

    @staticmethod
    def forward(ctx, t):
        c = t.shape[1] // 2
        ctx.c = c
        return t[:, :c], t[:, c:], t[:, c:]

    @staticmethod
    def backward(ctx, d0, d1a, d1b):
        L, st, c = lib(), stream(), ctx.c
        ref = next(g for g in (d0, d1a, d1b) if g is not None)
        dtype, dev = ref.dtype, ref.device
        B, _, H, W = ref.shape
        dt = code(dtype)
        esz = ref.element_size()
        P = B * H * W
        ok = lambda g: g is not None and g.dtype == dtype and is_nhwc(g) and g.data_ptr() % 16 == 0 and g.stride(3) % ce(dtype) == 0 and px_dense(g)
        if (d0 is not None and d1a is not None and ok(d0) and ok(d1a) and d0.stride() == d1a.stride()
                and d1a.data_ptr() == d0.data_ptr() + c * esz and d0.stride(3) >= 2 * c):
            if d1b is not None:
                d1b = to_nhwc(d1b, dtype, dense=True)
                L.add2d(dt, d1a.data_ptr(), d1a.stride(3), d1b.data_ptr(), d1b.stride(3), d1a.data_ptr(), d1a.stride(3), P, c, st)
            return torch.as_strided(d0, (B, 2 * c, H, W), d0.stride(), d0.storage_offset())
        out = nhwc_empty(B, 2 * c, H, W, dtype, dev)
        if d0 is None:
            out[:, :c].zero_()
        else:
            d0 = to_nhwc(d0, dtype, dense=True)
            L.copy2d(dt, d0.data_ptr(), d0.stride(3), out.data_ptr(), 2 * c, P, c, st)
        parts = [to_nhwc(g, dtype, dense=True) for g in (d1a, d1b) if g is not None]
        if not parts:
            out[:, c:].zero_()
        elif len(parts) == 1:
            L.copy2d(dt, parts[0].data_ptr(), parts[0].stride(3), out.data_ptr() + c * esz, 2 * c, P, c, st)
        else:
            L.add2d(dt, parts[0].data_ptr(), parts[0].stride(3), parts[1].data_ptr(), parts[1].stride(3), out.data_ptr() + c * esz, 2 * c, P, c, st)
        return out


class HeadProjFn(torch.autograd.Function):

    @staticmethod
    def forward(ctx, n, *args):
        L = lib()
        xs, ws, bs = args[:n], args[n:2 * n], args[2 * n:3 * n]
        dtype = _COMPUTE_DTYPE
        dt = code(dtype)
        st = stream()
        B, _, H, W = xs[0].shape
        P = B * H * W
        couts = [w.shape[0] for w in ws]
        tot = sum(couts)
        out = nhwc_empty(B, tot, H, W, dtype, xs[0].device)
        esz = out.element_size()
        xs = [to_nhwc(x, dtype, dense=True) for x in xs]
        w32 = [w.detach().float().contiguous() for w in ws]
        b32 = [b.detach().float().contiguous() for b in bs]
        off = 0
        wide = []
        for x, w, b, co in zip(xs, w32, b32, couts):
            Cin = x.shape[1]
            mf = co >= 32 and co % 8 == 0 and off % 8 == 0 and tot % 8 == 0 and Cin % 8 == 0
            wide.append(mf)
            if mf:
                wp = torch.empty(co * Cin, dtype=dtype, device=x.device)
                L.pack_weight_fwd(dt, w.data_ptr(), wp.data_ptr(), co, Cin, Cin, 1, 1, st)
                sb, sh, sw = s3(x)
                L.conv2d_fwd(dt, x.data_ptr(), sb, sh, sw, B, H, W, Cin, wp.data_ptr(), b.data_ptr(), out.data_ptr() + off * esz, tot, H, W, co,
                             1, 1, 1, 1, 0, None, st)
            else:
                for o0 in range(0, co, 24):
                    oc = min(24, co - o0)
                    L.proj_fwd(dt, x.data_ptr(), x.stride(3), w.data_ptr() + o0 * w.shape[1] * 4, b.data_ptr() + o0 * 4,
                               out.data_ptr() + (off + o0) * esz, tot, P, x.shape[1], oc, st)
            off += co
        ctx.n, ctx.couts, ctx.dtype, ctx.wide = n, couts, dtype, wide
        ctx.save_for_backward(*xs, *w32)
        return out

    @staticmethod
    def backward(ctx, dout):
        L = lib()
        n, couts, dtype = ctx.n, ctx.couts, ctx.dtype
        xs, ws = ctx.saved_tensors[:n], ctx.saved_tensors[n:]
        dt = code(dtype)
        st = stream()
        if not (dout.dtype == dtype and px_dense(dout)):
            dout = to_nhwc(dout, dtype, dense=True) if dout.shape[1] % ce(dtype) == 0 else _dense_any(dout, dtype)
        B, tot, H, W = dout.shape
        P = B * H * W
        dev = dout.device
        esz = dout.element_size()
        dsw = dout.stride(3)
        nb = L.proj_blocks(P)
        dxs, dws, dbs = [], [], []
        off = 0
        for j, (x, w, co) in enumerate(zip(xs, ws, couts)):
            Cin = x.shape[1]
            dx = None
            if ctx.wide[j]:
                dptr = dout.data_ptr() + off * esz
                dsb, dsh, _ = s3(dout)
                if ctx.needs_input_grad[1 + j]:
                    kp = L.conv_kpad(dt, co)
                    wpd = torch.empty(Cin * kp, dtype=dtype, device=dev)
                    L.pack_weight_dgrad(dt, w.data_ptr(), wpd.data_ptr(), co, Cin, 1, 1, 1, st)
                    dx = nhwc_empty(B, Cin, H, W, dtype, dev)
                    L.conv2d_bwd_data(dt, dptr, dsb, dsh, dsw, B, H, W, co, wpd.data_ptr(), dx.data_ptr(), Cin, H, W, Cin, 1, 1, 1, 1, 0, st)
                sb, sh, sw = s3(x)
                ns = L.conv2d_wgrad_plan(dt, B, H, W, Cin, co, 1, 1, 1, 1, 0)
                slab = _f32(ns * co * Cin, dev)
                dW = torch.empty_like(w)
                L.conv2d_bwd_weight(dt, x.data_ptr(), sb, sh, sw, B, H, W, Cin, Cin, dptr, dsw, H, W, co, 1, 1, 1, 1, 0, slab.data_ptr(), ns,
                                    dW.data_ptr(), 0, st)
                nbb = L.bn_bwd_blocks(P, co)
                part = _f32(nbb * co * 2, dev)
                L.colsum_partials(dt, dptr, dsw, part.data_ptr(), P, co, st)
                db, scratch = _f32(co, dev), _f32(2 * co, dev)
                L.bn_bwd_finalize(part.data_ptr(), nbb, co, P, None, db.data_ptr(), 0, scratch.data_ptr(), scratch.data_ptr() + 4 * co, st)
                dxs.append(dx)
                dws.append(dW)
                dbs.append(db)
                off += co
                continue
            if ctx.needs_input_grad[1 + j]:
                dx = nhwc_empty(B, Cin, H, W, dtype, dev)
                first = True
                for o0 in range(0, co, 24):
                    oc = min(24, co - o0)
                    if first:
                        L.proj_bwd_data(dt, dout.data_ptr() + (off + o0) * esz, dsw, w.data_ptr() + o0 * Cin * 4, dx.data_ptr(), Cin, P, Cin, oc, st)
                        first = False
                    else:
                        tmp = nhwc_empty(B, Cin, H, W, dtype, dev)
                        L.proj_bwd_data(dt, dout.data_ptr() + (off + o0) * esz, dsw, w.data_ptr() + o0 * Cin * 4, tmp.data_ptr(), Cin, P, Cin, oc, st)
                        L.add2d(dt, dx.data_ptr(), Cin, tmp.data_ptr(), Cin, dx.data_ptr(), Cin, P, Cin, st)
            dW = torch.empty_like(w)
            db = _f32(co, dev)
            slab = _f32(nb * co * Cin, dev)
            bslab = _f32(nb * co, dev)
            L.proj_bwd_weight(dt, x.data_ptr(), x.stride(3), dout.data_ptr() + off * esz, dsw, slab.data_ptr(), bslab.data_ptr(),
                              dW.data_ptr(), db.data_ptr(), 0, P, Cin, co, st)
            dxs.append(dx)
            dws.append(dW)
            dbs.append(db)
            off += co
        return (None, *dxs, *dws, *dbs)


def proj_slices_eval(x, offsets, cin, ws, bs):
    import ctypes
    n = len(ws)
    dtype = _COMPUTE_DTYPE
    if not (dtype == torch.bfloat16 and cin in (64, 128) and PROJ_BN_MFMA and n <= 16):
        return HeadProjSlicesFn.apply(x, offsets, [cin] * n, n, *ws, *bs)
    L, st = lib(), stream()
    x = to_nhwc(x, dtype, dense=True)
    B, Ct, H, W = x.shape
    couts = [w.shape[0] for w in ws]
    tot = sum(couts)
    out = nhwc_empty(B, tot, H, W, dtype, x.device)
    w32 = [w.detach().float().contiguous() for w in ws]
    b32 = [b.detach().float().contiguous() for b in bs]
    ident = _identity_bn(Ct, x.device)
    PV, IA = ctypes.c_void_p * n, ctypes.c_int * n
    L.proj_group_fwd_bn_mfma(n, cin, x.data_ptr(), x.stride(3), IA(*offsets), PV(*[t.data_ptr() for t in w32]), PV(*[t.data_ptr() for t in b32]), IA(*couts),
                             ident[0].data_ptr(), ident[1].data_ptr(), 0, out.data_ptr(), tot, B * H * W, st)
    return out


class HeadProjSlicesFn(torch.autograd.Function):

    @staticmethod
    def forward(ctx, x, offsets, cins, n, *args):
        import ctypes
        L = lib()
        ws, bs = args[:n], args[n:2 * n]
        dtype = _COMPUTE_DTYPE
        dt = code(dtype)
        st = stream()
        x = to_nhwc(x, dtype, dense=True)
        B, Ct, H, W = x.shape
        P = B * H * W
        couts = [w.shape[0] for w in ws]
        cin = cins[0]
        assert all(c == cin for c in cins) and n <= 16, "HeadProjSlicesFn: uniform branch width, at most 16 branches"
        tot = sum(couts)
        out = nhwc_empty(B, tot, H, W, dtype, x.device)
        w32 = [w.detach().float().contiguous() for w in ws]
        b32 = [b.detach().float().contiguous() for b in bs]
        PV = ctypes.c_void_p * n
        IA = ctypes.c_int * n
        c_w, c_b = PV(*[w.data_ptr() for w in w32]), PV(*[b.data_ptr() for b in b32])
        c_off, c_co = IA(*offsets), IA(*couts)
        L.proj_group_fwd(dt, n, cin, x.data_ptr(), x.stride(3), c_off, c_w, c_b, c_co, out.data_ptr(), tot, P, st)
        ctx.meta = (list(offsets), cin, n, couts, dtype)
        ctx.save_for_backward(x, *w32)
        return out

    @staticmethod
    def backward(ctx, dout):
        import ctypes
        L = lib()
        offsets, cin, n, couts, dtype = ctx.meta
        x, ws = ctx.saved_tensors[0], ctx.saved_tensors[1:]
        dt = code(dtype)
        st = stream()
        if not (dout.dtype == dtype and px_dense(dout)):
            dout = _dense_any(dout, dtype)
        B, Ct, H, W = x.shape
        P = B * H * W
        dev = x.device
        tot = sum(couts)
        PV = ctypes.c_void_p * n
        IA = ctypes.c_int * n
        c_w, c_off, c_co = PV(*[w.data_ptr() for w in ws]), IA(*offsets), IA(*couts)
        dx = None
        if ctx.needs_input_grad[0]:
            dx = nhwc_empty(B, Ct, H, W, dtype, dev)
            if n * cin != Ct:
                dx.zero_()
            L.proj_group_bwd_data(dt, n, cin, dout.data_ptr(), dout.stride(3), c_off, c_w, c_co, dx.data_ptr(), Ct, P, st)
        dws = [torch.empty_like(w) for w in ws]
        dbs = [_f32(co, dev) for co in couts]
        nb = L.proj_group_blocks(P)
        slab = _f32(nb * tot * cin, dev)
        bslab = _f32(nb * tot, dev)
        L.proj_group_bwd_weight(dt, n, cin, x.data_ptr(), x.stride(3), c_off, dout.data_ptr(), dout.stride(3), c_co, slab.data_ptr(),
                                bslab.data_ptr(), PV(*[t.data_ptr() for t in dws]), PV(*[t.data_ptr() for t in dbs]), P, st)
        return (dx, None, None, None, *dws, *dbs)


class FusedConvBNProjFn(torch.autograd.Function):

    @staticmethod
    def forward(ctx, x, stack, groups, offsets, cins, n, *params):
        import ctypes
        L = lib()
        w, gm, bt, rm, rv = stack.tensors()
        m = stack.convs[0]
        npar = len(params) - 2 * n
        ws, bs = params[npar:npar + n], params[npar + n:]
        ctx.gslot = grad_slot(x) if (m.training and x.is_cuda) else None
        y, cfg, saved = _cba_forward(x, w, gm, bt, rm, rv, m.k, m.s, m.p, groups, m.has_act, None, 0, m.training, m.eps, m.momentum, bn_apply=False,
                                     ver=stack.ver)
        if m.training:
            for c in stack.convs:
                c._nbt_pending += 1
        dtype = _COMPUTE_DTYPE
        dt, st = code(dtype), stream()
        B, Ct, H, W = y.shape
        P = B * H * W
        couts = [t.shape[0] for t in ws]
        cin = cins[0]
        assert all(c == cin for c in cins) and n <= 16 and n * cin == Ct and cin % 64 == 0
        tot = sum(couts)
        out = nhwc_empty(B, tot, H, W, dtype, y.device)
        w32 = [t.detach().float().contiguous() for t in ws]
        b32 = [t.detach().float().contiguous() for t in bs]
        PV, IA = ctypes.c_void_p * n, ctypes.c_int * n
        stats = saved[3]
        if dtype == torch.bfloat16 and cin in (64, 128) and PROJ_BN_MFMA:
            L.proj_group_fwd_bn_mfma(n, cin, y.data_ptr(), y.stride(3), IA(*offsets), PV(*[t.data_ptr() for t in w32]), PV(*[t.data_ptr() for t in b32]),
                                     IA(*couts), stats[2].data_ptr(), stats[3].data_ptr(), int(m.has_act), out.data_ptr(), tot, P, st)
        else:
            L.proj_group_fwd_bn(dt, n, cin, y.data_ptr(), y.stride(3), IA(*offsets), PV(*[t.data_ptr() for t in w32]), PV(*[t.data_ptr() for t in b32]),
                                IA(*couts), stats[2].data_ptr(), stats[3].data_ptr(), int(m.has_act), out.data_ptr(), tot, P, st)
        ctx.cfg, ctx.couts_stack, ctx.meta = cfg, stack.couts, (list(offsets), cin, n, couts, dtype, int(m.has_act))
        ctx.nsaved = len(saved)
        ctx.save_for_backward(*[t for t in saved if t is not None], *w32)
        ctx.none_mask = [t is None for t in saved]
        return out

    @staticmethod
    def backward(ctx, dout):
        import ctypes
        L = lib()
        offsets, cin, n, couts, dtype, act = ctx.meta
        it = iter(ctx.saved_tensors)
        saved = tuple(None if isnone else next(it) for isnone in ctx.none_mask)
        ws = list(it)
        xin, w32c, y, stats, _ = saved
        dt, st = code(dtype), stream()
        if not (dout.dtype == dtype and px_dense(dout)):
            dout = _dense_any(dout, dtype)
        B, Ct, H, W = y.shape
        P = B * H * W
        dev = y.device
        tot = sum(couts)
        PV, IA = ctypes.c_void_p * n, ctypes.c_int * n
        c_w, c_off, c_co = PV(*[t.data_ptr() for t in ws]), IA(*offsets), IA(*couts)
        dws = [torch.empty_like(t) for t in ws]
        dbs = [_f32(co, dev) for co in couts]
        mfma = dtype == torch.bfloat16 and cin in (64, 128) and PROJ_BN_MFMA
        dx_out = grad_slot_tensor(ctx.gslot) if (ctx.gslot is not None and ctx.needs_input_grad[0]) else None
        nb = L.proj_group_bwd_weight_bn_mfma_blocks(P) if mfma else L.proj_group_blocks(P)
        slab, bslab = _f32(nb * tot * cin, dev), _f32(nb * tot, dev)
        if mfma:
            L.proj_group_bwd_weight_bn_mfma(n, cin, y.data_ptr(), y.stride(3), c_off, dout.data_ptr(), dout.stride(3), c_co, stats[2].data_ptr(),
                                            stats[3].data_ptr(), act, slab.data_ptr(), bslab.data_ptr(), PV(*[t.data_ptr() for t in dws]),
                                            PV(*[t.data_ptr() for t in dbs]), P, st)
        else:
            L.proj_group_bwd_weight_bn(dt, n, cin, y.data_ptr(), y.stride(3), c_off, dout.data_ptr(), dout.stride(3), c_co, stats[2].data_ptr(),
                                       stats[3].data_ptr(), act, slab.data_ptr(), bslab.data_ptr(), PV(*[t.data_ptr() for t in dws]),
                                       PV(*[t.data_ptr() for t in dbs]), P, st)
        if mfma and ctx.cfg.training:
            nblk = L.proj_group_bn_bwd_blocks(P)
            part = _f32(nblk * Ct * 2, dev)
            args = (n, cin, y.data_ptr(), y.stride(3), c_off, dout.data_ptr(), dout.stride(3), c_w, c_co, stats[2].data_ptr(), stats[3].data_ptr(),
                    stats[0].data_ptr(), stats[1].data_ptr())
            L.proj_group_bn_bwd(0, *args, None, None, act, part.data_ptr(), nblk, None, 0, P, Ct, st)
            dgb = _f32(2 * Ct, dev).view(2, Ct)
            L.bn_bwd_finalize(part.data_ptr(), nblk, Ct, P, dgb[0].data_ptr(), dgb[1].data_ptr(), 0, stats[4].data_ptr(), stats[5].data_ptr(), st)
            dy = nhwc_empty(B, Ct, H, W, dtype, dev)
            L.proj_group_bn_bwd(1, *args, stats[4].data_ptr(), stats[5].data_ptr(), act, None, 0, dy.data_ptr(), Ct, P, Ct, st)
            dx, dW, dg, db, _ = _cba_backward(ctx.cfg, saved, None, ctx.needs_input_grad[0], False, None, pre=(dy, dgb), dx_out=dx_out)
        else:
            dz = nhwc_empty(B, Ct, H, W, dtype, dev)
            L.proj_group_bwd_data(dt, n, cin, dout.data_ptr(), dout.stride(3), c_off, c_w, c_co, dz.data_ptr(), Ct, P, st)
            dx, dW, dg, db, _ = _cba_backward(ctx.cfg, saved, dz, ctx.needs_input_grad[0], False, None, dx_out=dx_out)
        dWs, dgs, dbs_s, off = [], [], [], 0
        for co in ctx.couts_stack:
            dWs.append(dW[off:off + co])
            dgs.append(dg[off:off + co])
            dbs_s.append(db[off:off + co])
            off += co
        return (dx, None, None, None, None, None, *dWs, *dgs, *dbs_s, *dws, *dbs)


def _dense_any(x, dtype):
    B, C, H, W = x.shape
    out = nhwc_empty(B, C, H, W, dtype, x.device)
    out.copy_(x)
    return out


class ConcatFn(torch.autograd.Function):

    @staticmethod
    def forward(ctx, *xs):
        L = lib()
        dtype = _COMPUTE_DTYPE
        dt = code(dtype)
        st = stream()
        B, _, H, W = xs[0].shape
        cs = [x.shape[1] for x in xs]
        tot = sum(cs)
        ctx.cs = cs
        esz = 2 if dtype == torch.bfloat16 else 4
        out, inplace, off = None, [False] * len(xs), 0
        for i, (x, c) in enumerate(zip(xs, cs)):
            if (PLACEMENT and x.dtype == dtype and x.is_cuda and is_nhwc(x) and x.stride(3) == tot and x.stride(2) == W * tot
                    and x.stride(0) == H * W * tot):
                base = x.data_ptr() - off * esz
                if out is None and _CONCAT_BASE.get(base, (None, None))[0] == tot:
                    del _CONCAT_BASE[base]
                    out = torch.as_strided(x, (B, tot, H, W), x.stride(), x.storage_offset() - off)
                    assert out.data_ptr() == base
                    inplace[i] = True
                elif out is not None and out.data_ptr() == base:
                    inplace[i] = True
            off += c
        if out is None:
            out = nhwc_empty(B, tot, H, W, dtype, xs[0].device)
        off = 0
        for i, (x, c) in enumerate(zip(xs, cs)):
            if not inplace[i]:
                x = to_nhwc(x, dtype, dense=True)
                L.copy2d(dt, x.data_ptr(), x.stride(3), out.data_ptr() + off * esz, tot, B * H * W, c, st)
            off += c
        return out

    @staticmethod
    def backward(ctx, dout):
        outs, off = [], 0
        for c in ctx.cs:
            outs.append(dout[:, off:off + c])
            off += c
        return tuple(outs)


class MaxPoolFn(torch.autograd.Function):

    @staticmethod
    def forward(ctx, x, k):
        L = lib()
        dtype = _COMPUTE_DTYPE
        dt = code(dtype)
        x = to_nhwc(x, dtype)
        B, C, H, W = x.shape
        y = out_tensor(B, C, H, W, dtype, x.device)
        need = x.requires_grad
        arg = torch.empty(B * H * W * C, dtype=torch.uint8, device=x.device) if need else None
        sb, sh, sw = s3(x)
        L.maxpool_fwd(dt, x.data_ptr(), sb, sh, sw, y.data_ptr(), y.stride(3), arg.data_ptr() if need else None, B, H, W, C, k, stream())
        ctx.k = k
        ctx.dtype = dtype
        if need:
            ctx.save_for_backward(arg)
        return y

    @staticmethod
    def backward(ctx, dy):
        L = lib()
        (arg,) = ctx.saved_tensors
        dtype = ctx.dtype
        dy = to_nhwc(dy, dtype, dense=True)
        B, C, H, W = dy.shape
        dx = nhwc_empty(B, C, H, W, dtype, dy.device)
        L.maxpool_bwd(code(dtype), dy.data_ptr(), dy.stride(3), arg.data_ptr(), dx.data_ptr(), C, B, H, W, C, ctx.k, stream())
        return dx, None


class Upsample2xFn(torch.autograd.Function):

    @staticmethod
    def forward(ctx, x):
        L = lib()
        dtype = _COMPUTE_DTYPE
        x = to_nhwc(x, dtype)
        B, C, H, W = x.shape
        y = out_tensor(B, C, 2 * H, 2 * W, dtype, x.device)
        sb, sh, sw = s3(x)
        L.upsample2x_fwd(code(dtype), x.data_ptr(), sb, sh, sw, y.data_ptr(), y.stride(3), B, H, W, C, stream())
        ctx.dtype = dtype
        return y

    @staticmethod
    def backward(ctx, dy):
        L = lib()
        dtype = ctx.dtype
        dy = to_nhwc(dy, dtype)
        B, C, H2, W2 = dy.shape
        dx = nhwc_empty(B, C, H2 // 2, W2 // 2, dtype, dy.device)
        sb, sh, sw = s3(dy)
        L.upsample2x_bwd(code(dtype), dy.data_ptr(), sb, sh, sw, dx.data_ptr(), C, B, H2 // 2, W2 // 2, C, stream())
        return dx


class AttentionFn(torch.autograd.Function):

    @staticmethod
    def forward(ctx, qkv, nh, kd, hd, scale):
        L = lib()
        dtype = _COMPUTE_DTYPE
        dt = code(dtype)
        st = stream()
        qkv = to_nhwc(qkv, dtype, dense=True)
        B, Ct, H, W = qkv.shape
        N = H * W
        C = nh * hd
        dev = qkv.device
        out = nhwc_empty(B, C, H, W, dtype, dev)
        v = nhwc_empty(B, C, H, W, dtype, dev)
        lse = _f32(B * nh * N, dev)
        L.attn_fwd(dt, qkv.data_ptr(), qkv.stride(3), out.data_ptr(), C, lse.data_ptr(), B, N, nh, kd, hd, scale, st)
        esz = qkv.element_size()
        for h in range(nh):
            L.copy2d(dt, qkv.data_ptr() + (h * (2 * kd + hd) + 2 * kd) * esz, qkv.stride(3), v.data_ptr() + h * hd * esz, C, B * N, hd, st)
        ctx.cfg = (nh, kd, hd, scale, dtype)
        ctx.save_for_backward(qkv, out, lse)
        return out, v

    @staticmethod
    def backward(ctx, dout, dv):
        L = lib()
        qkv, out, lse = ctx.saved_tensors
        nh, kd, hd, scale, dtype = ctx.cfg
        dt = code(dtype)
        B, Ct, H, W = qkv.shape
        N = H * W
        C = nh * hd
        dev = qkv.device
        if dout is None:
            dout = torch.zeros_like(out)
        dout = to_nhwc(dout, dtype, dense=True)
        dvp, dvs = None, 0
        if dv is not None:
            dv = to_nhwc(dv, dtype, dense=True)
            dvp, dvs = dv.data_ptr(), dv.stride(3)
        dqkv = nhwc_empty(B, Ct, H, W, dtype, dev)
        delta = _f32(B * nh * N, dev)
        L.attn_bwd(dt, qkv.data_ptr(), qkv.stride(3), out.data_ptr(), C, dout.data_ptr(), dout.stride(3), dvp, dvs, lse.data_ptr(),
                   delta.data_ptr(), dqkv.data_ptr(), Ct, B, N, nh, kd, hd, scale, stream())
        return dqkv, None, None, None, None
```

Baseline: 1415.

## Add LDS-tiled depthwise conv kernels for forward, dgrad and wgrad

```diff
diff --git a/include/y3d.h b/include/y3d.h
--- a/include/y3d.h
+++ b/include/y3d.h
@@ -87,6 +87,23 @@
 int y3d_dwconv2d_bwd_data(int dtype, const void* dy, int64_t dsb, int64_t dsh, int64_t dsw, int B, int Ho, int Wo, int C,
                           const float* w_packed, void* dx, int64_t xsw, int H, int W, int kh, int kw, int stride, int pad,
                           void* stream);
+int y3d_set_dw_tiled(int enable);
+int y3d_get_dw_tiled(void);
+int y3d_dw_plan_tiled(int B, int H, int W, int C, int k, int stride, int dgrad);
+int y3d_dw_plan_rows(int B, int H, int W, int C, int k, int stride);
+int y3d_dw_plan_strip_rows(int B, int H, int W, int C, int k, int stride, int dgrad);
+int y3d_dw_plan_lds(int B, int H, int W, int C, int k, int stride, int dgrad);
+int y3d_dwconv2d_fwd_oihw(int dtype, const void* x, int64_t xsb, int64_t xsh, int64_t xsw, int B, int H, int W, int C,
+                          const float* w_oihw, void* y, int64_t ysw, int Ho, int Wo, int kh, int kw, int stride, int pad,
+                          float* stat_partials, int partial_rows, void* stream);
+int y3d_dwconv2d_bwd_data_oihw(int dtype, const void* dy, int64_t dsb, int64_t dsh, int64_t dsw, int B, int Ho, int Wo, int C,
+                               const float* w_oihw, void* dx, int64_t xsw, int H, int W, int kh, int kw, int stride, int pad,
+                               void* stream);
+int y3d_dw_plan_wgrad_rows(int B, int H, int W, int C, int k, int stride);
+int y3d_dw_plan_wgrad_tiled(int B, int H, int W, int C, int k, int stride);
+int y3d_dwconv2d_bwd_weight_rows(int dtype, const void* x, int64_t xsb, int64_t xsh, int64_t xsw, int B, int H, int W, int C,
+                                 const void* dy, int64_t dsw, int Ho, int Wo, int kh, int kw, int stride, int pad, float* slab,
+                                 int slab_rows, float* grad_oihw, int accumulate, void* stream);
 int y3d_dwconv2d_bwd_weight(int dtype, const void* x, int64_t xsb, int64_t xsh, int64_t xsw, int B, int H, int W, int C,
                             const void* dy, int64_t dsw, int Ho, int Wo, int kh, int kw, int stride, int pad, float* slab,
                             float* grad_oihw, int accumulate, void* stream);
diff --git a/yolov10-3d_amd/_lib.py b/yolov10-3d_amd/_lib.py
--- a/yolov10-3d_amd/_lib.py
+++ b/yolov10-3d_amd/_lib.py
@@ -37,7 +37,7 @@
     return protos
 
 
-_PLAIN_INT = {"abi_version", "conv_kpad", "conv_stat_blocks", "conv2d_stat_rows", "conv2d_route", "conv2d_wgrad_splits", "conv2d_wgrad_plan", "set_tile_kernels", "set_stream1x1", "set_bn_wide_slabs", "get_stream1x1", "get_tile_kernels", "dw_blocks", "dw_wgrad_blocks", "bn_bwd_blocks", "proj_blocks", "proj_group_blocks", "proj_group_bn_bwd_blocks", "proj_group_bwd_weight_bn_mfma_blocks", "tal3d_scratch_floats", "tal2d_scratch_floats", "v10_postprocess_scratch_floats", "conv2d_fwd_affine_res_ok", "stem_conv_train_rows", "conv3x3_fp8_ok", "conv3x3_fp8_dgrad_ok", "conv3x3_fp8_stat_rows", "fp8_scale_pitch", "kitti_eval_max_boxes", "det_metrics_max_gts", "det_metrics_max_dets"}
+_PLAIN_INT = {"abi_version", "conv_kpad", "conv_stat_blocks", "conv2d_stat_rows", "conv2d_route", "conv2d_wgrad_splits", "conv2d_wgrad_plan", "set_tile_kernels", "set_stream1x1", "set_bn_wide_slabs", "get_stream1x1", "get_tile_kernels", "dw_blocks", "dw_wgrad_blocks", "set_dw_tiled", "get_dw_tiled", "dw_plan_tiled", "dw_plan_rows", "dw_plan_strip_rows", "dw_plan_lds", "dw_plan_wgrad_rows", "dw_plan_wgrad_tiled", "bn_bwd_blocks", "proj_blocks", "proj_group_blocks", "proj_group_bn_bwd_blocks", "proj_group_bwd_weight_bn_mfma_blocks", "tal3d_scratch_floats", "tal2d_scratch_floats", "v10_postprocess_scratch_floats", "conv2d_fwd_affine_res_ok", "stem_conv_train_rows", "conv3x3_fp8_ok", "conv3x3_fp8_dgrad_ok", "conv3x3_fp8_stat_rows", "fp8_scale_pitch", "kitti_eval_max_boxes", "det_metrics_max_gts", "det_metrics_max_dets"}
 
 
 class _Lib:
diff --git a/yolov10-3d_amd/csrc/dwconv.hip b/yolov10-3d_amd/csrc/dwconv.hip
--- a/yolov10-3d_amd/csrc/dwconv.hip
+++ b/yolov10-3d_amd/csrc/dwconv.hip
@@ -17,12 +17,14 @@
 struct DwP {
   const void* x;
   const float* w;
+  long wts, wcs;
   void* y;
   float* part;
   long xsb, xsh, xsw, ysw;
   int B, Hg, Wg, Hq, Wq, C, kh, kw, stride, pad;
   long M;
   int px_per_block;
+  int TR, RPR, Hh, Wh, strips, cap;
   const float *scale, *shift;
   const void* res;
   long rsw;
@@ -43,7 +45,7 @@
   const int c = cs + ct * CE;
   for (int i = threadIdx.x; i < taps * 64; i += 256) {
     int t = i / 64, cc = i % 64;
-    sw[i] = (cs + cc < p.C) ? p.w[(long)t * p.C + cs + cc] : 0.f;
+    sw[i] = (cs + cc < p.C) ? p.w[(long)t * p.wts + (cs + cc) * p.wcs] : 0.f;
   }
   __syncthreads();
   const T* __restrict__ X = (const T*)p.x;
@@ -168,6 +170,168 @@
   }
 }
 
+template <int K, int S, bool DGRAD, bool AFF>
+__global__ __launch_bounds__(256) void dwconv_tiled_kernel(DwP p) {
+  typedef bf16_t T;
+  constexpr int CE = 8;
+  constexpr bool D2 = DGRAD && S == 2;
+  constexpr int R = D2 ? 4 : 5;
+  constexpr int NI = D2 ? 3 : S * (R - 1) + K;
+  constexpr int RS = D2 ? 2 : S * R;
+  extern __shared__ __attribute__((aligned(16))) char smem[];
+  float* sw = (float*)smem;
+  float* sred = sw + K * K * 64;
+  char* halo = (char*)(sred + 4 * 64 * 2);
+  const int tid = threadIdx.x, ct = tid & 7, slot = tid >> 3;
+  const int cs = blockIdx.y * 64, c = cs + ct * CE;
+  const int b = blockIdx.x / p.strips, strip = blockIdx.x - b * p.strips;
+  const int h0 = strip * p.TR;
+  const int rows = h0 + p.TR < p.Hq ? p.TR : p.Hq - h0;
+  for (int i = tid; i < K * K * 64; i += 256) {
+    const int t = p.wcs == 1 ? i >> 6 : i % (K * K), cc = p.wcs == 1 ? i & 63 : i / (K * K);
+    sw[t * 64 + cc] = (cs + cc < p.C) ? p.w[(long)t * p.wts + (cs + cc) * p.wcs] : 0.f;
+  }
+  {
+    const int gh0 = D2 ? h0 / 2 : (DGRAD ? h0 + p.pad - (K - 1) : S * h0 - p.pad);
+    const int gw0 = D2 ? 0 : (DGRAD ? p.pad - (K - 1) : -p.pad);
+    const T* __restrict__ xb = (const T*)p.x + (long)b * p.xsb + c;
+    const bool cok = c < p.C;
+    const int npos = p.Hh * p.Wh;
+    int pos = slot;
+    int row = pos / p.Wh, col = pos - row * p.Wh;
+    for (; pos < npos; pos += 32 * 4) {
+      uint4 v[4];
+#pragma unroll
+      for (int u = 0; u < 4; ++u) {
+        const int gh = gh0 + row, gw = gw0 + col;
+        const bool ok = cok && pos + 32 * u < npos && gh >= 0 && gh < p.Hg && gw >= 0 && gw < p.Wg;
+        v[u] = ok ? *(const uint4*)(xb + (long)gh * p.xsh + (long)gw * p.xsw) : make_uint4(0, 0, 0, 0);
+        col += 32;
+        while (col >= p.Wh) { col -= p.Wh; ++row; }
+      }
+#pragma unroll
+      for (int u = 0; u < 4; ++u)
+        if (pos + 32 * u < npos) *(uint4*)(halo + (long)(pos + 32 * u) * 128 + ct * 16) = v[u];
+    }
+  }
+  __syncthreads();
+  float s1[CE], s2[CE];
+#pragma unroll
+  for (int j = 0; j < CE; ++j) { s1[j] = 0.f; s2[j] = 0.f; }
+  float esc[CE], esf[CE];
+  if (AFF && c < p.C) {
+#pragma unroll
+    for (int j = 0; j < CE; ++j) { esc[j] = p.scale[c + j]; esf[j] = p.shift[c + j]; }
+  }
+  T* __restrict__ Y = (T*)p.y;
+  const int nruns = rows * p.RPR;
+  int hl = slot / p.RPR, cr = slot - hl * p.RPR;
+  for (int n = slot; n < nruns; n += 32) {
+    float acc[R][CE];
+#pragma unroll
+    for (int j = 0; j < R; ++j)
+#pragma unroll
+      for (int e = 0; e < CE; ++e) acc[j][e] = 0.f;
+    if constexpr (D2) {
+      const int odd = hl & 1;
+      for (int rr = 0; rr <= odd; ++rr) {
+        const int r = odd ? 2 * rr : 1;
+        const int lrow = odd ? (hl + 1) / 2 - rr : hl / 2;
+        float wr[3][CE];
+#pragma unroll
+        for (int q = 0; q < 3; ++q) {
+          *(float4*)&wr[q][0] = *(const float4*)(sw + (r * 3 + q) * 64 + ct * CE);
+          *(float4*)&wr[q][4] = *(const float4*)(sw + (r * 3 + q) * 64 + ct * CE + 4);
+        }
+        const char* rp = halo + ((long)(lrow * p.Wh + RS * cr) * 128 + ct * 16);
+        float v0[CE], v1[CE], v2[CE];
+        Chunk<T>::unpack(*(const uint4*)(rp), v0);
+        Chunk<T>::unpack(*(const uint4*)(rp + 128), v1);
+        Chunk<T>::unpack(*(const uint4*)(rp + 256), v2);
+        pk_fma<CE>(acc[0], v0, wr[1]);
+        pk_fma<CE>(acc[1], v1, wr[0]);
+        pk_fma<CE>(acc[1], v0, wr[2]);
+        pk_fma<CE>(acc[2], v1, wr[1]);
+        pk_fma<CE>(acc[3], v2, wr[0]);
+        pk_fma<CE>(acc[3], v1, wr[2]);
+      }
+    } else {
+#pragma unroll 1
+      for (int r = 0; r < K; ++r) {
+        float wr[K][CE];
+#pragma unroll
+        for (int q = 0; q < K; ++q) {
+          *(float4*)&wr[q][0] = *(const float4*)(sw + (r * K + q) * 64 + ct * CE);
+          *(float4*)&wr[q][4] = *(const float4*)(sw + (r * K + q) * 64 + ct * CE + 4);
+        }
+        const int lrow = DGRAD ? hl + (K - 1) - r : S * hl + r;
+        const char* rp = halo + ((long)(lrow * p.Wh + RS * cr) * 128 + ct * 16);
+#pragma unroll
+        for (int ii = 0; ii < NI; ++ii) {
+          const int i = DGRAD ? NI - 1 - ii : ii;
+          float v[CE];
+          Chunk<T>::unpack(*(const uint4*)(rp + i * 128), v);
+#pragma unroll
+          for (int j = 0; j < R; ++j) {
+            const int q = DGRAD ? j + (K - 1) - i : i - S * j;
+            if (q >= 0 && q < K) pk_fma<CE>(acc[j], v, wr[q]);
+          }
+        }
+      }
+    }
+    if (c < p.C) {
+      const int w0 = R * cr;
+      const long mrow = ((long)b * p.Hq + h0 + hl) * p.Wq;
+#pragma unroll
+      for (int j = 0; j < R; ++j) {
+        if (w0 + j >= p.Wq) break;
+        const long m = mrow + w0 + j;
+#pragma unroll
+        for (int e = 0; e < CE; ++e) {
+          acc[j][e] = TT<T>::rnd(acc[j][e]);
+          s1[e] += acc[j][e];
+          s2[e] += acc[j][e] * acc[j][e];
+        }
+        if (AFF) {
+          float rv[CE];
+          if (p.res_mode) Chunk<T>::unpack(*(const uint4*)((const T*)p.res + m * p.rsw + c), rv);
+#pragma unroll
+          for (int e = 0; e < CE; ++e) {
+            float u = acc[j][e] * esc[e] + esf[e];
+            if (p.res_mode == 2) u += rv[e];
+            if (p.act) u = silu_f(u);
+            if (p.res_mode == 1) u += rv[e];
+            acc[j][e] = u;
+          }
+        }
+        *(uint4*)(Y + m * p.ysw + c) = Chunk<T>::pack(acc[j]);
+      }
+    }
+    cr += 32;
+    while (cr >= p.RPR) { cr -= p.RPR; ++hl; }
+  }
+  if (p.part) {
+    const int lane = tid & 63, wave = tid >> 6;
+#pragma unroll
+    for (int e = 0; e < CE; ++e) {
+      const float a = lane_xor32_sum(lane_xor16_sum(lane_xor8_sum(s1[e])));
+      const float q = lane_xor32_sum(lane_xor16_sum(lane_xor8_sum(s2[e])));
+      if (lane < 8) { sred[(wave * 64 + ct * CE + e) * 2] = a; sred[(wave * 64 + ct * CE + e) * 2 + 1] = q; }
+    }
+    __syncthreads();
+    if (tid < 64 && cs + tid < p.C) {
+      const float a = (sred[tid * 2] + sred[(64 + tid) * 2]) + (sred[(128 + tid) * 2] + sred[(192 + tid) * 2]);
+      const float q = (sred[tid * 2 + 1] + sred[(64 + tid) * 2 + 1]) + (sred[(128 + tid) * 2 + 1] + sred[(192 + tid) * 2 + 1]);
+      p.part[((long)blockIdx.x * p.C + cs + tid) * 2] = a;
+      p.part[((long)blockIdx.x * p.C + cs + tid) * 2 + 1] = q;
+      for (long rw = (long)gridDim.x + blockIdx.x; rw < p.cap; rw += gridDim.x) {
+        p.part[(rw * p.C + cs + tid) * 2] = 0.f;
+        p.part[(rw * p.C + cs + tid) * 2 + 1] = 0.f;
+      }
+    }
+  }
+}
+
 struct DwWP {
   const void* x;
   const void* dy;
@@ -176,6 +340,7 @@
   int B, H, W, Ho, Wo, C, kh, kw, stride, pad;
   long M;
   int px_per_block, nblk, nslab;
+  int TR, RPR, DW, Hh, Wh, strips;
 };
 
 template <typename T, int K>
@@ -277,6 +442,102 @@
   }
 }
 
+template <int K>
+__global__ __launch_bounds__(256) void dwconv_wgrad_tiled_kernel(DwWP p) {
+  typedef bf16_t T;
+  constexpr int CE = 8, R = 5, NI = R + K - 1;
+  extern __shared__ __attribute__((aligned(16))) char smem[];
+  char* sdy = smem;
+  char* sx = smem + (long)p.TR * p.DW * 128;
+  const int tid = threadIdx.x, ct = tid & 7, slot = tid >> 3, lane = tid & 63, wave = tid >> 6;
+  const int cs = blockIdx.y * 64, c = cs + ct * CE;
+  const int b = blockIdx.x / p.strips, strip = blockIdx.x - b * p.strips;
+  const int h0 = strip * p.TR;
+  const int rows = h0 + p.TR < p.Ho ? p.TR : p.Ho - h0;
+  const bool cok = c < p.C;
+  {
+    const T* __restrict__ db = (const T*)p.dy + ((long)b * p.Ho + h0) * p.Wo * p.dsw + c;
+    const int npos = p.TR * p.DW;
+    int pos = slot;
+    int row = pos / p.DW, col = pos - row * p.DW;
+    for (; pos < npos; pos += 32 * 4) {
+      uint4 v[4];
+#pragma unroll
+      for (int u = 0; u < 4; ++u) {
+        const bool ok = cok && pos + 32 * u < npos && row < rows && col < p.Wo;
+        v[u] = ok ? *(const uint4*)(db + ((long)row * p.Wo + col) * p.dsw) : make_uint4(0, 0, 0, 0);
+        col += 32;
+        while (col >= p.DW) { col -= p.DW; ++row; }
+      }
+#pragma unroll
+      for (int u = 0; u < 4; ++u)
+        if (pos + 32 * u < npos) *(uint4*)(sdy + (long)(pos + 32 * u) * 128 + ct * 16) = v[u];
+    }
+  }
+  {
+    const T* __restrict__ xb = (const T*)p.x + (long)b * p.xsb + c;
+    const int gh0 = h0 - p.pad, gw0 = -p.pad;
+    const int npos = p.Hh * p.Wh;
+    int pos = slot;
+    int row = pos / p.Wh, col = pos - row * p.Wh;
+    for (; pos < npos; pos += 32 * 4) {
+      uint4 v[4];
+#pragma unroll
+      for (int u = 0; u < 4; ++u) {
+        const int gh = gh0 + row, gw = gw0 + col;
+        const bool ok = cok && pos + 32 * u < npos && gh >= 0 && gh < p.H && gw >= 0 && gw < p.W;
+        v[u] = ok ? *(const uint4*)(xb + (long)gh * p.xsh + (long)gw * p.xsw) : make_uint4(0, 0, 0, 0);
+        col += 32;
+        while (col >= p.Wh) { col -= p.Wh; ++row; }
+      }
+#pragma unroll
+      for (int u = 0; u < 4; ++u)
+        if (pos + 32 * u < npos) *(uint4*)(sx + (long)(pos + 32 * u) * 128 + ct * 16) = v[u];
+    }
+  }
+  __syncthreads();
+  const int s8 = slot & 7;
+  const int nruns = rows * p.RPR;
+  for (int r = wave; r < K; r += 4) {
+    float acc[K][CE];
+#pragma unroll
+    for (int q = 0; q < K; ++q)
+#pragma unroll
+      for (int e = 0; e < CE; ++e) acc[q][e] = 0.f;
+    int hl = s8 / p.RPR, cr = s8 - hl * p.RPR;
+    for (int n = s8; n < nruns; n += 8) {
+      const char* dp = sdy + ((long)(hl * p.DW + R * cr) * 128 + ct * 16);
+      const char* xp = sx + ((long)((hl + r) * p.Wh + R * cr) * 128 + ct * 16);
+      float d[R][CE];
+#pragma unroll
+      for (int j = 0; j < R; ++j) Chunk<T>::unpack(*(const uint4*)(dp + j * 128), d[j]);
+#pragma unroll
+      for (int i = 0; i < NI; ++i) {
+        float v[CE];
+        Chunk<T>::unpack(*(const uint4*)(xp + i * 128), v);
+#pragma unroll
+        for (int j = 0; j < R; ++j) {
+          const int q = i - j;
+          if (q >= 0 && q < K) pk_fma<CE>(acc[q], d[j], v);
+        }
+      }
+      cr += 8;
+      while (cr >= p.RPR) { cr -= p.RPR; ++hl; }
+    }
+#pragma unroll
+    for (int q = 0; q < K; ++q) {
+      float o[CE];
+#pragma unroll
+      for (int e = 0; e < CE; ++e) o[e] = lane_xor32_sum(lane_xor16_sum(lane_xor8_sum(acc[q][e])));
+      if (lane < 8 && cok) {
+        float* dst = p.slab + ((long)blockIdx.x * (K * K) + r * K + q) * p.C + c;
+        *(float4*)dst = make_float4(o[0], o[1], o[2], o[3]);
+        *(float4*)(dst + 4) = make_float4(o[4], o[5], o[6], o[7]);
+      }
+    }
+  }
+}
+
 __global__ __launch_bounds__(256) void dw_wgrad_reduce_kernel(const float* __restrict__ slab, float* __restrict__ grad, int nblk, int taps, int C,
                                                               int accumulate) {
   __shared__ float sh[8][32];
@@ -333,12 +594,68 @@
     else { if (kk == 3) DW_LAUNCH_K(T, false, 3); else if (kk == 7) DW_LAUNCH_K(T, false, 7); else DW_LAUNCH_K(T, false, 0); }        \
   } while (0)
 
-static int dw_launch(int dtype, bool dgrad, const DwP& p, hipStream_t st) {
+static int g_dw_tiled = 1;
+
+struct DwTile {
+  int ok, TR, RPR, Hh, Wh, strips;
+  long tiles;
+  size_t lds;
+};
+constexpr size_t DW_TILE_LDS = 64 * 1024;
+
+static DwTile dw_tile_plan(int dtype, int B, int Hq, int Wq, int kh, int kw, int stride, int pad, bool dgrad) {
+  DwTile t = {};
+  if (dtype != Y3D_BF16 || kh != kw || pad != kh / 2 || B < 1 || Hq < 1 || Wq < 1) return t;
+  if (!((kh == 3 && (stride == 1 || (stride == 2 && dgrad))) || (kh == 7 && stride == 1))) return t;
+  const int K = kh, S = stride;
+  const bool d2 = dgrad && S == 2;
+  const int R = d2 ? 4 : 5;
+  t.RPR = (Wq + R - 1) / R;
+  t.Wh = d2 ? 2 * t.RPR + 1 : S * (R * t.RPR - 1) + K;
+  const size_t fixed = (size_t)(K * K * 64 + 4 * 64 * 2) * sizeof(float);
+  auto halo_rows = [&](int tr) { return d2 ? tr / 2 + 1 : S * (tr - 1) + K; };
+  auto fits = [&](int tr) { return fixed + (size_t)halo_rows(tr) * t.Wh * 128 <= DW_TILE_LDS; };
+  const int step = d2 ? 2 : 1, want = d2 ? 128 : 32;
+  int tr = step;
+  if (!fits(tr)) return t;
+  while (tr * t.RPR < want && tr < Hq && fits(tr + step)) tr += step;
+  int strips = (Hq + tr - 1) / tr;
+  tr = (Hq + strips - 1) / strips;
+  if (d2 && (tr & 1)) ++tr;
+  if (!fits(tr)) return t;
+  t.TR = tr;
+  t.strips = (Hq + tr - 1) / tr;
+  t.Hh = halo_rows(tr);
+  t.tiles = (long)B * t.strips;
+  t.lds = fixed + (size_t)t.Hh * t.Wh * 128;
+  if (t.tiles > y3d_dw_blocks((long)B * Hq * Wq)) return t;
+  t.ok = 1;
+  return t;
+}
+
+#define DW_TILED(K, S, D, A) hipLaunchKernelGGL((dwconv_tiled_kernel<K, S, D, A>), grid, dim3(256), t.lds, st, p)
+
+static int dw_launch(int dtype, bool dgrad, DwP& p, int cap, hipStream_t st) {
   Y3D_CHECK(p.M < (1L << 31), "dwconv: more than 2^31 pixels");
+  const DwTile t = g_dw_tiled ? dw_tile_plan(dtype, p.B, p.Hq, p.Wq, p.kh, p.kw, p.stride, p.pad, dgrad) : DwTile{};
+  if (t.ok) {
+    Y3D_CHECK(!p.part || t.tiles <= cap, "dwconv: %ld rows of partials needed, %d given", t.tiles, cap);
+    p.TR = t.TR; p.RPR = t.RPR; p.Hh = t.Hh; p.Wh = t.Wh; p.strips = t.strips; p.cap = cap;
+    dim3 grid((unsigned)t.tiles, cdiv(p.C, 64));
+    const bool aff = !dgrad && p.scale;
+    if (p.kh == 7) { if (dgrad) DW_TILED(7, 1, true, false); else if (aff) DW_TILED(7, 1, false, true); else DW_TILED(7, 1, false, false); }
+    else if (p.stride == 1) { if (dgrad) DW_TILED(3, 1, true, false); else if (aff) DW_TILED(3, 1, false, true); else DW_TILED(3, 1, false, false); }
+    else DW_TILED(3, 2, true, false);
+    Y3D_LAUNCH_CHECK();
+    return Y3D_OK;
+  }
+  const int nblk = y3d_dw_blocks(p.M);
+  Y3D_CHECK(!p.part || nblk <= cap, "dwconv: %d rows of partials needed, %d given", nblk, cap);
+  p.px_per_block = (int)((p.M + nblk - 1) / nblk);
   int ce = dtype == Y3D_BF16 ? 8 : 4;
   int pt = 256 / (64 / ce);
   size_t sm = (size_t)(p.kh * p.kw * 64 + pt * 64 * 2) * sizeof(float);
-  dim3 grid(y3d_dw_blocks(p.M), cdiv(p.C, 64));
+  dim3 grid(nblk, cdiv(p.C, 64));
   if (dtype == Y3D_BF16) {
     DW_LAUNCH(bf16_t);
   } else {
@@ -348,67 +665,151 @@
   return Y3D_OK;
 }
 
+int y3d_set_dw_tiled(int enable) {
+  const int old = g_dw_tiled;
+  g_dw_tiled = enable ? 1 : 0;
+  return old;
+}
+int y3d_get_dw_tiled(void) { return g_dw_tiled; }
+
+int y3d_dw_plan_tiled(int B, int H, int W, int C, int k, int stride, int dgrad) {
+  const int Ho = (H + 2 * (k / 2) - k) / stride + 1, Wo = (W + 2 * (k / 2) - k) / stride + 1;
+  (void)C;
+  return g_dw_tiled ? dw_tile_plan(Y3D_BF16, B, dgrad ? H : Ho, dgrad ? W : Wo, k, k, stride, k / 2, dgrad != 0).ok : 0;
+}
+int y3d_dw_plan_rows(int B, int H, int W, int C, int k, int stride) {
+  const int Ho = (H + 2 * (k / 2) - k) / stride + 1, Wo = (W + 2 * (k / 2) - k) / stride + 1;
+  (void)C;
+  const DwTile t = g_dw_tiled ? dw_tile_plan(Y3D_BF16, B, Ho, Wo, k, k, stride, k / 2, false) : DwTile{};
+  return t.ok ? (int)t.tiles : y3d_dw_blocks((long)B * Ho * Wo);
+}
+int y3d_dw_plan_strip_rows(int B, int H, int W, int C, int k, int stride, int dgrad) {
+  const int Ho = (H + 2 * (k / 2) - k) / stride + 1, Wo = (W + 2 * (k / 2) - k) / stride + 1;
+  (void)C;
+  const DwTile t = g_dw_tiled ? dw_tile_plan(Y3D_BF16, B, dgrad ? H : Ho, dgrad ? W : Wo, k, k, stride, k / 2, dgrad != 0) : DwTile{};
+  return t.ok ? t.TR : 0;
+}
+int y3d_dw_plan_lds(int B, int H, int W, int C, int k, int stride, int dgrad) {
+  const int Ho = (H + 2 * (k / 2) - k) / stride + 1, Wo = (W + 2 * (k / 2) - k) / stride + 1;
+  (void)C;
+  const DwTile t = g_dw_tiled ? dw_tile_plan(Y3D_BF16, B, dgrad ? H : Ho, dgrad ? W : Wo, k, k, stride, k / 2, dgrad != 0) : DwTile{};
+  return t.ok ? (int)t.lds : 0;
+}
+
+static int dw_fwd(const char* who, int dtype, const void* x, int64_t xsb, int64_t xsh, int64_t xsw, int B, int H, int W, int C, const float* w, long wts,
+                  long wcs, const float* scale, const float* shift, int act, int res_mode, const void* res, int64_t rsw, void* y, int64_t ysw, int Ho,
+                  int Wo, int kh, int kw, int stride, int pad, float* part, int cap, void* stream) {
+  int ce = dtype == Y3D_BF16 ? 8 : 4;
+  Y3D_CHECK(dtype == Y3D_BF16 || dtype == Y3D_F32, "%s: bad dtype", who);
+  Y3D_CHECK(C % ce == 0, "%s: C=%d not a multiple of %d", who, C, ce);
+  Y3D_CHECK(Ho == (H + 2 * pad - kh) / stride + 1 && Wo == (W + 2 * pad - kw) / stride + 1, "%s: output dims", who);
+  Y3D_CHECK((((uintptr_t)x | (uintptr_t)y) & 15) == 0 && xsb % ce == 0 && xsh % ce == 0 && xsw % ce == 0 && ysw % ce == 0, "%s: alignment", who);
+  DwP p;
+  p.x = x; p.w = w; p.wts = wts; p.wcs = wcs; p.y = y; p.part = part;
+  p.scale = scale; p.shift = shift; p.res = res; p.rsw = rsw; p.act = act; p.res_mode = res_mode;
+  p.xsb = xsb; p.xsh = xsh; p.xsw = xsw; p.ysw = ysw;
+  p.B = B; p.Hg = H; p.Wg = W; p.Hq = Ho; p.Wq = Wo; p.C = C; p.kh = kh; p.kw = kw; p.stride = stride; p.pad = pad;
+  p.M = (long)B * Ho * Wo;
+  return dw_launch(dtype, false, p, cap, (hipStream_t)stream);
+}
+
+static int dw_bwd_data(const char* who, int dtype, const void* dy, int64_t dsb, int64_t dsh, int64_t dsw, int B, int Ho, int Wo, int C, const float* w,
+                       long wts, long wcs, void* dx, int64_t xsw, int H, int W, int kh, int kw, int stride, int pad, void* stream) {
+  int ce = dtype == Y3D_BF16 ? 8 : 4;
+  Y3D_CHECK(dtype == Y3D_BF16 || dtype == Y3D_F32, "%s: bad dtype", who);
+  Y3D_CHECK(C % ce == 0, "%s: C=%d not a multiple of %d", who, C, ce);
+  Y3D_CHECK((((uintptr_t)dy | (uintptr_t)dx) & 15) == 0 && dsb % ce == 0 && dsh % ce == 0 && dsw % ce == 0 && xsw % ce == 0, "%s: alignment", who);
+  DwP p;
+  p.x = dy; p.w = w; p.wts = wts; p.wcs = wcs; p.y = dx; p.part = nullptr;
+  p.scale = nullptr; p.shift = nullptr; p.res = nullptr; p.rsw = 0; p.act = 0; p.res_mode = 0;
+  p.xsb = dsb; p.xsh = dsh; p.xsw = dsw; p.ysw = xsw;
+  p.B = B; p.Hg = Ho; p.Wg = Wo; p.Hq = H; p.Wq = W; p.C = C; p.kh = kh; p.kw = kw; p.stride = stride; p.pad = pad;
+  p.M = (long)B * H * W;
+  return dw_launch(dtype, true, p, 0, (hipStream_t)stream);
+}
+
 int y3d_dwconv2d_fwd(int dtype, const void* x, int64_t xsb, int64_t xsh, int64_t xsw, int B, int H, int W, int C,
                      const float* w_packed, void* y, int64_t ysw, int Ho, int Wo, int kh, int kw, int stride, int pad,
                      float* stat_partials, void* stream) {
-  int ce = dtype == Y3D_BF16 ? 8 : 4;
-  Y3D_CHECK(dtype == Y3D_BF16 || dtype == Y3D_F32, "dwconv2d_fwd: bad dtype");
-  Y3D_CHECK(C % ce == 0, "dwconv2d_fwd: C=%d not a multiple of %d", C, ce);
-  Y3D_CHECK(Ho == (H + 2 * pad - kh) / stride + 1 && Wo == (W + 2 * pad - kw) / stride + 1, "dwconv2d_fwd: output dims");
-  Y3D_CHECK((((uintptr_t)x | (uintptr_t)y) & 15) == 0 && xsb % ce == 0 && xsh % ce == 0 && xsw % ce == 0 && ysw % ce == 0, "dwconv2d_fwd: alignment");
-  DwP p;
-  p.x = x; p.w = w_packed; p.y = y; p.part = stat_partials;
-  p.scale = nullptr; p.shift = nullptr; p.res = nullptr; p.rsw = 0; p.act = 0; p.res_mode = 0;
-  p.xsb = xsb; p.xsh = xsh; p.xsw = xsw; p.ysw = ysw;
-  p.B = B; p.Hg = H; p.Wg = W; p.Hq = Ho; p.Wq = Wo; p.C = C; p.kh = kh; p.kw = kw; p.stride = stride; p.pad = pad;
-  p.M = (long)B * Ho * Wo;
-  int nblk = y3d_dw_blocks(p.M);
-  p.px_per_block = (int)((p.M + nblk - 1) / nblk);
-  return dw_launch(dtype, false, p, (hipStream_t)stream);
+  return dw_fwd("dwconv2d_fwd", dtype, x, xsb, xsh, xsw, B, H, W, C, w_packed, C, 1, nullptr, nullptr, 0, 0, nullptr, 0, y, ysw, Ho, Wo, kh, kw, stride,
+                pad, stat_partials, y3d_dw_blocks((long)B * Ho * Wo), stream);
+}
+
+int y3d_dwconv2d_fwd_oihw(int dtype, const void* x, int64_t xsb, int64_t xsh, int64_t xsw, int B, int H, int W, int C,
+                          const float* w_oihw, void* y, int64_t ysw, int Ho, int Wo, int kh, int kw, int stride, int pad,
+                          float* stat_partials, int partial_rows, void* stream) {
+  return dw_fwd("dwconv2d_fwd_oihw", dtype, x, xsb, xsh, xsw, B, H, W, C, w_oihw, 1, (long)kh * kw, nullptr, nullptr, 0, 0, nullptr, 0, y, ysw, Ho, Wo,
+                kh, kw, stride, pad, stat_partials, partial_rows, stream);
 }
 
 int y3d_dwconv2d_fwd_affine(int dtype, const void* x, int64_t xsb, int64_t xsh, int64_t xsw, int B, int H, int W, int C,
                             const float* w_packed, const float* scale, const float* shift, int act, int res_mode, const void* res, int64_t rsw,
                             void* z, int64_t zsw, int Ho, int Wo, int kh, int kw, int stride, int pad, void* stream) {
   int ce = dtype == Y3D_BF16 ? 8 : 4;
-  Y3D_CHECK(dtype == Y3D_BF16 || dtype == Y3D_F32, "dwconv2d_fwd_affine: bad dtype");
-  Y3D_CHECK(C % ce == 0, "dwconv2d_fwd_affine: C=%d not a multiple of %d", C, ce);
-  Y3D_CHECK(Ho == (H + 2 * pad - kh) / stride + 1 && Wo == (W + 2 * pad - kw) / stride + 1, "dwconv2d_fwd_affine: output dims");
-  Y3D_CHECK((((uintptr_t)x | (uintptr_t)z) & 15) == 0 && xsb % ce == 0 && xsh % ce == 0 && xsw % ce == 0 && zsw % ce == 0, "dwconv2d_fwd_affine: alignment");
   Y3D_CHECK(scale && shift && res_mode >= 0 && res_mode <= 2, "dwconv2d_fwd_affine: scale / shift missing or bad residual mode");
   Y3D_CHECK(res_mode == 0 || (res && (((uintptr_t)res) & 15) == 0 && rsw % ce == 0), "dwconv2d_fwd_affine: residual missing or misaligned");
-  DwP p;
-  p.x = x; p.w = w_packed; p.y = z; p.part = nullptr;
-  p.scale = scale; p.shift = shift; p.res = res; p.rsw = rsw; p.act = act; p.res_mode = res_mode;
-  p.xsb = xsb; p.xsh = xsh; p.xsw = xsw; p.ysw = zsw;
-  p.B = B; p.Hg = H; p.Wg = W; p.Hq = Ho; p.Wq = Wo; p.C = C; p.kh = kh; p.kw = kw; p.stride = stride; p.pad = pad;
-  p.M = (long)B * Ho * Wo;
-  int nblk = y3d_dw_blocks(p.M);
-  p.px_per_block = (int)((p.M + nblk - 1) / nblk);
-  return dw_launch(dtype, false, p, (hipStream_t)stream);
+  return dw_fwd("dwconv2d_fwd_affine", dtype, x, xsb, xsh, xsw, B, H, W, C, w_packed, C, 1, scale, shift, act, res_mode, res, rsw, z, zsw, Ho, Wo, kh, kw,
+                stride, pad, nullptr, 0, stream);
 }
 
 int y3d_dwconv2d_bwd_data(int dtype, const void* dy, int64_t dsb, int64_t dsh, int64_t dsw, int B, int Ho, int Wo, int C,
                           const float* w_packed, void* dx, int64_t xsw, int H, int W, int kh, int kw, int stride, int pad,
                           void* stream) {
-  int ce = dtype == Y3D_BF16 ? 8 : 4;
-  Y3D_CHECK(dtype == Y3D_BF16 || dtype == Y3D_F32, "dwconv2d_bwd_data: bad dtype");
-  Y3D_CHECK(C % ce == 0, "dwconv2d_bwd_data: C=%d not a multiple of %d", C, ce);
-  Y3D_CHECK((((uintptr_t)dy | (uintptr_t)dx) & 15) == 0 && dsb % ce == 0 && dsh % ce == 0 && dsw % ce == 0 && xsw % ce == 0, "dwconv2d_bwd_data: alignment");
-  DwP p;
-  p.x = dy; p.w = w_packed; p.y = dx; p.part = nullptr;
-  p.scale = nullptr; p.shift = nullptr; p.res = nullptr; p.rsw = 0; p.act = 0; p.res_mode = 0;
-  p.xsb = dsb; p.xsh = dsh; p.xsw = dsw; p.ysw = xsw;
-  p.B = B; p.Hg = Ho; p.Wg = Wo; p.Hq = H; p.Wq = W; p.C = C; p.kh = kh; p.kw = kw; p.stride = stride; p.pad = pad;
-  p.M = (long)B * H * W;
-  int nblk = y3d_dw_blocks(p.M);
-  p.px_per_block = (int)((p.M + nblk - 1) / nblk);
-  return dw_launch(dtype, true, p, (hipStream_t)stream);
-}
-
-int y3d_dwconv2d_bwd_weight(int dtype, const void* x, int64_t xsb, int64_t xsh, int64_t xsw, int B, int H, int W, int C,
-                            const void* dy, int64_t dsw, int Ho, int Wo, int kh, int kw, int stride, int pad, float* slab,
-                            float* grad_oihw, int accumulate, void* stream) {
+  return dw_bwd_data("dwconv2d_bwd_data", dtype, dy, dsb, dsh, dsw, B, Ho, Wo, C, w_packed, C, 1, dx, xsw, H, W, kh, kw, stride, pad, stream);
+}
+
+int y3d_dwconv2d_bwd_data_oihw(int dtype, const void* dy, int64_t dsb, int64_t dsh, int64_t dsw, int B, int Ho, int Wo, int C,
+                               const float* w_oihw, void* dx, int64_t xsw, int H, int W, int kh, int kw, int stride, int pad,
+                               void* stream) {
+  return dw_bwd_data("dwconv2d_bwd_data_oihw", dtype, dy, dsb, dsh, dsw, B, Ho, Wo, C, w_oihw, 1, (long)kh * kw, dx, xsw, H, W, kh, kw, stride, pad,
+                     stream);
+}
+
+struct DwWTile {
+  int ok, TR, RPR, DW, Hh, Wh, strips;
+  long tiles;
+  size_t lds;
+};
+static DwWTile dw_wgrad_tile_plan(int dtype, int B, int Ho, int Wo, int kh, int kw, int stride, int pad) {
+  DwWTile t = {};
+  if (dtype != Y3D_BF16 || kh != kw || (kh != 3 && kh != 7) || stride != 1 || pad != kh / 2 || B < 1 || Ho < 1 || Wo < 1) return t;
+  const int K = kh, R = 5;
+  t.RPR = (Wo + R - 1) / R;
+  t.DW = R * t.RPR;
+  t.Wh = t.DW + K - 1;
+  auto lds = [&](int tr) { return ((size_t)tr * t.DW + (size_t)(tr + K - 1) * t.Wh) * 128; };
+  int tr = 1;
+  if (lds(tr) > DW_TILE_LDS) return t;
+  while (tr < Ho && lds(tr + 1) <= DW_TILE_LDS && (tr + 1 <= 8 || (long)B * ((Ho + tr) / (tr + 1)) >= 96)) ++tr;
+  const int strips = (Ho + tr - 1) / tr;
+  tr = (Ho + strips - 1) / strips;
+  t.TR = tr;
+  t.strips = strips;
+  t.Hh = tr + K - 1;
+  t.tiles = (long)B * strips;
+  t.lds = lds(tr);
+  if (tr < 2 && Ho > 1) return t;
+  t.ok = 1;
+  return t;
+}
+
+int y3d_dw_plan_wgrad_rows(int B, int H, int W, int C, int k, int stride) {
+  const int Ho = (H + 2 * (k / 2) - k) / stride + 1, Wo = (W + 2 * (k / 2) - k) / stride + 1;
+  (void)C;
+  const DwWTile t = g_dw_tiled ? dw_wgrad_tile_plan(Y3D_BF16, B, Ho, Wo, k, k, stride, k / 2) : DwWTile{};
+  const int old = y3d_dw_wgrad_blocks((long)B * Ho * Wo);
+  return t.ok && t.tiles <= old ? (int)t.tiles : old;
+}
+int y3d_dw_plan_wgrad_tiled(int B, int H, int W, int C, int k, int stride) {
+  const int Ho = (H + 2 * (k / 2) - k) / stride + 1, Wo = (W + 2 * (k / 2) - k) / stride + 1;
+  (void)C;
+  const DwWTile t = g_dw_tiled ? dw_wgrad_tile_plan(Y3D_BF16, B, Ho, Wo, k, k, stride, k / 2) : DwWTile{};
+  return t.ok && t.tiles <= y3d_dw_wgrad_blocks((long)B * Ho * Wo) ? (int)t.lds : 0;
+}
+
+static int dw_bwd_weight(int dtype, const void* x, int64_t xsb, int64_t xsh, int64_t xsw, int B, int H, int W, int C, const void* dy, int64_t dsw,
+                         int Ho, int Wo, int kh, int kw, int stride, int pad, float* slab, int slab_rows, float* grad_oihw, int accumulate,
+                         void* stream) {
   int ce = dtype == Y3D_BF16 ? 8 : 4;
   Y3D_CHECK(dtype == Y3D_BF16 || dtype == Y3D_F32, "dwconv2d_bwd_weight: bad dtype");
   Y3D_CHECK(C % ce == 0, "dwconv2d_bwd_weight: C=%d not a multiple of %d", C, ce);
@@ -418,24 +819,49 @@
   p.xsb = xsb; p.xsh = xsh; p.xsw = xsw; p.dsw = dsw;
   p.B = B; p.H = H; p.W = W; p.Ho = Ho; p.Wo = Wo; p.C = C; p.kh = kh; p.kw = kw; p.stride = stride; p.pad = pad;
   p.M = (long)B * Ho * Wo;
-  int nblk = y3d_dw_wgrad_blocks(p.M);
-  p.px_per_block = (int)((p.M + nblk - 1) / nblk);
-  p.nblk = nblk; p.nslab = cdiv(C, 64);
-  dim3 grid(cdiv(nblk * p.nslab, 8) * 8 * kh);
   hipStream_t st = (hipStream_t)stream;
   Y3D_CHECK(kw <= 8 || (kh == kw && (kh == 3 || kh == 7)), "dwconv2d_bwd_weight: kernels wider than 8 taps are not supported");
+  int nblk = y3d_dw_wgrad_blocks(p.M);
+  const DwWTile t = g_dw_tiled && Ho == (H + 2 * pad - kh) / stride + 1 && Wo == (W + 2 * pad - kw) / stride + 1 && (((uintptr_t)slab) & 15) == 0
+                        ? dw_wgrad_tile_plan(dtype, B, Ho, Wo, kh, kw, stride, pad) : DwWTile{};
+  if (t.ok && t.tiles <= nblk) {
+    nblk = (int)t.tiles;
+    Y3D_CHECK(nblk <= slab_rows, "dwconv2d_bwd_weight: %d slab rows needed, %d given", nblk, slab_rows);
+    p.TR = t.TR; p.RPR = t.RPR; p.DW = t.DW; p.Hh = t.Hh; p.Wh = t.Wh; p.strips = t.strips;
+    dim3 grid((unsigned)t.tiles, cdiv(C, 64));
+    if (kh == 3) hipLaunchKernelGGL((dwconv_wgrad_tiled_kernel<3>), grid, dim3(256), t.lds, st, p);
+    else hipLaunchKernelGGL((dwconv_wgrad_tiled_kernel<7>), grid, dim3(256), t.lds, st, p);
+  } else {
+    Y3D_CHECK(nblk <= slab_rows, "dwconv2d_bwd_weight: %d slab rows needed, %d given", nblk, slab_rows);
+    p.px_per_block = (int)((p.M + nblk - 1) / nblk);
+    p.nblk = nblk; p.nslab = cdiv(C, 64);
+    dim3 grid(cdiv(nblk * p.nslab, 8) * 8 * kh);
 #define Y3D_DWW(T)                                                                                                          \
   do {                                                                                                                      \
     if (kh == 3 && kw == 3) hipLaunchKernelGGL((dwconv_wgrad_kernel<T, 3>), grid, dim3(256), 0, st, p);                      \
     else if (kh == 7 && kw == 7) hipLaunchKernelGGL((dwconv_wgrad_kernel<T, 7>), grid, dim3(256), 0, st, p);                 \
     else hipLaunchKernelGGL((dwconv_wgrad_kernel<T, 0>), grid, dim3(256), 0, st, p);                                         \
   } while (0)
-  if (dtype == Y3D_BF16) Y3D_DWW(bf16_t); else Y3D_DWW(float);
+    if (dtype == Y3D_BF16) Y3D_DWW(bf16_t); else Y3D_DWW(float);
 #undef Y3D_DWW
+  }
   Y3D_LAUNCH_CHECK();
   hipLaunchKernelGGL(dw_wgrad_reduce_kernel, dim3(cdiv((long)C * kh * kw, 32)), dim3(256), 0, st, slab, grad_oihw, nblk, kh * kw, C, accumulate);
   Y3D_LAUNCH_CHECK();
   return Y3D_OK;
 }
 
-}
+int y3d_dwconv2d_bwd_weight(int dtype, const void* x, int64_t xsb, int64_t xsh, int64_t xsw, int B, int H, int W, int C,
+                            const void* dy, int64_t dsw, int Ho, int Wo, int kh, int kw, int stride, int pad, float* slab,
+                            float* grad_oihw, int accumulate, void* stream) {
+  return dw_bwd_weight(dtype, x, xsb, xsh, xsw, B, H, W, C, dy, dsw, Ho, Wo, kh, kw, stride, pad, slab, y3d_dw_wgrad_blocks((long)B * Ho * Wo), grad_oihw,
+                       accumulate, stream);
+}
+
+int y3d_dwconv2d_bwd_weight_rows(int dtype, const void* x, int64_t xsb, int64_t xsh, int64_t xsw, int B, int H, int W, int C,
+                                 const void* dy, int64_t dsw, int Ho, int Wo, int kh, int kw, int stride, int pad, float* slab,
+                                 int slab_rows, float* grad_oihw, int accumulate, void* stream) {
+  return dw_bwd_weight(dtype, x, xsb, xsh, xsw, B, H, W, C, dy, dsw, Ho, Wo, kh, kw, stride, pad, slab, slab_rows, grad_oihw, accumulate, stream);
+}
+
+}
diff --git a/yolov10-3d_amd/ops.py b/yolov10-3d_amd/ops.py
--- a/yolov10-3d_amd/ops.py
+++ b/yolov10-3d_amd/ops.py
@@ -601,12 +601,13 @@
     sb, sh, sw = s3(xin)
     fused = not training and bn_apply and DW_EVAL_FUSED
     y = None if fused else nhwc_empty(B, C, Ho, Wo, dtype, dev)
-    nblk = L.dw_blocks(B * Ho * Wo)
     part = ss_eval = None
     if training:
+        nblk = L.dw_plan_rows(B, H, W, C, k, s) if (p == k // 2 and dtype == torch.bfloat16) else L.dw_blocks(B * Ho * Wo)
         part = _f32(nblk * C * 2, dev)
-        wp = _f32(k * k * C, dev)
-        L.dw_pack_weight(w32.data_ptr(), wp.data_ptr(), C, k, k, st)
+        L.dwconv2d_fwd_oihw(dt, xin.data_ptr(), sb, sh, sw, B, H, W, C, w32.data_ptr(), y.data_ptr(), C, Ho, Wo, k, k, s, p, part.data_ptr(), nblk, st)
+        return _bn_act_tail(xin, w32, y, part, nblk, None, g32, b32, rm, rv, C, k, s, p, C, act, res, res_mode, training, eps, momentum, bn_apply,
+                            ver[0] if ver is not None else None, None)
     else:
         wp, ss_eval = _eval_consts(cache, "dw", w32, g32, b32, rm, rv, ver, dtype, k, C, 1, 1, C, eps)
         if fused:
@@ -618,9 +619,8 @@
                                   res_mode, rr.data_ptr() if rr is not None else None, rr.stride(3) if rr is not None else 0,
                                   ze.data_ptr(), ze.stride(3), Ho, Wo, k, k, s, p, st)
             return ze, None, None
-    L.dwconv2d_fwd(dt, xin.data_ptr(), sb, sh, sw, B, H, W, C, wp.data_ptr(), y.data_ptr(), C, Ho, Wo, k, k, s, p,
-                   part.data_ptr() if training else None, st)
-    return _bn_act_tail(xin, w32, y, part, nblk, ss_eval, g32, b32, rm, rv, C, k, s, p, C, act, res, res_mode, training, eps, momentum, bn_apply,
+    L.dwconv2d_fwd(dt, xin.data_ptr(), sb, sh, sw, B, H, W, C, wp.data_ptr(), y.data_ptr(), C, Ho, Wo, k, k, s, p, None, st)
+    return _bn_act_tail(xin, w32, y, None, 0, ss_eval, g32, b32, rm, rv, C, k, s, p, C, act, res, res_mode, training, eps, momentum, bn_apply,
                         ver[0] if ver is not None else None, None)
 
 
@@ -776,15 +776,14 @@
     dx = None
     dW = torch.empty_like(w32)
     if plan.dw:
-        wp = _f32(k * k * Cout, dev)
-        L.dw_pack_weight(w32.data_ptr(), wp.data_ptr(), Cout, k, k, st)
         if need_dx:
             dx = nhwc_empty(B, Cin, H, W, dtype, dev)
             dsb, dsh, dsw = s3(dy)
-            L.dwconv2d_bwd_data(dt, dy.data_ptr(), dsb, dsh, dsw, B, Ho, Wo, Cout, wp.data_ptr(), dx.data_ptr(), Cin, H, W, k, k, s, p, st)
-        slab = _f32(L.dw_wgrad_blocks(M) * k * k * Cout, dev)
-        L.dwconv2d_bwd_weight(dt, xin.data_ptr(), sb, sh, sw, B, H, W, Cin, dy.data_ptr(), Cout, Ho, Wo, k, k, s, p, slab.data_ptr(),
-                              dW.data_ptr(), 0, st)
+            L.dwconv2d_bwd_data_oihw(dt, dy.data_ptr(), dsb, dsh, dsw, B, Ho, Wo, Cout, w32.data_ptr(), dx.data_ptr(), Cin, H, W, k, k, s, p, st)
+        srows = L.dw_plan_wgrad_rows(B, H, W, Cin, k, s) if (p == k // 2 and dtype == torch.bfloat16) else L.dw_wgrad_blocks(M)
+        slab = _f32(srows * k * k * Cout, dev)
+        L.dwconv2d_bwd_weight_rows(dt, xin.data_ptr(), sb, sh, sw, B, H, W, Cin, dy.data_ptr(), Cout, Ho, Wo, k, k, s, p, slab.data_ptr(), srows,
+                                   dW.data_ptr(), 0, st)
     else:
         f8 = _fp8_dgrad_plan(plan, need_dx, dx_range)
         if f8 is not None and not (px_dense(dy) and dy.data_ptr() % 16 == 0 and dy.stride(3) % 8 == 0):
```

After: 1426 (median of 6 runs). About the same (+0.8%).
